# zhenpeiyang/RelativePose

Measured on AMD Instinct MI355X. Metric: scan-pairs/sec end-to-end (completion+feat+spectral-match), 160x640 RGB-D, higher is better.
Workload: dtype f32 (fp32 products emulated on the bf16 matrix pipe: every operand cut into 3 bf16 pieces = its full 24 significand bits, the 6 partial products >= 2^-16 |ab| issued as v_mfma_f32_32x32x16_bf16, the 3 smallest dropped: a product error <= 2^-23 |ab| worst case, rms 2^-27.4 -- an fp32 multiply's own r

## Files before the change

### include/relpose.h

```cpp
#ifndef RELPOSE_H
#define RELPOSE_H

#include <stddef.h>
#include <stdint.h>

#ifdef __cplusplus
extern "C" {
#endif

#define RELPOSE_EINVAL (-1)
#define RELPOSE_ENOMEM (-2)

enum {
    RELPOSE_OK = 0,
    RELPOSE_FEW_KEYPOINTS = 1,
    RELPOSE_DIST_FILTER = 2,
    RELPOSE_ANGLE_FILTER = 3,
    RELPOSE_ZERO_WEIGHT = 4,
    RELPOSE_EDGE_OVERFLOW = 5,
    RELPOSE_NOT_CONVERGED = 6
};

enum { RELPOSE_SUNCG = 0, RELPOSE_MATTERPORT = 1, RELPOSE_SCANNET = 2 };
enum { RELPOSE_MASK_SECOND = 0, RELPOSE_MASK_KINECT = 1 };
enum { RELPOSE_COMPOSE_EVAL = 0, RELPOSE_COMPOSE_LIB = 1 };
enum { RELPOSE_FIT_IRLS_SM = 0, RELPOSE_FIT_HORN87 = 1, RELPOSE_FIT_IRLS = 2, RELPOSE_FIT_SPECTRAL = 3 };

typedef struct RelposeParams {
    double distThre;
    double distSepThre;
    double angleThre;
    double sigmaAngle1, sigmaAngle2, sigmaDist, sigmaFeat;
    double mu;
    int32_t topK;
    int32_t method;
} RelposeParams;

void relpose_default_params(RelposeParams* p_host);

enum { RELPOSE_TUNE_AFFINITY_KERNEL = 0, RELPOSE_TUNE_FIT_MAX_PRODUCTS = 1, RELPOSE_TUNE_FIT_CLUSTER = 2,
       RELPOSE_TUNE_FIT_GLOBAL_VECTORS = 3, RELPOSE_TUNE_FIT_FIXED_CHECKS = 4, RELPOSE_TUNE_HEADS_KERNEL = 5, RELPOSE_TUNE_DECONV_STRIP = 6,
       RELPOSE_TUNE_ZERO_TILES = 7, RELPOSE_TUNE_CONV1_ZERO = 8, RELPOSE_TUNE_COUNT = 9 };
int relpose_set_tuning(int32_t key, int32_t value);
const char* relpose_version(void);
typedef struct RelposeKeypoints {
    int32_t B, ns_max, nt_max;
    const int32_t* ns;
    const int32_t* nt;
    const double* pc_s;
    const double* normal_s;
    const float* feat_s;
    const double* weight_s;
    const double* pc_t;
    const double* normal_t;
    const float* feat_t;
    const double* weight_t;
} RelposeKeypoints;

typedef struct RelposeMatchDebug {
    float* wij;
    int32_t* corres_j;
    double* corres_w;
    int32_t* counts;
    double* trace;
    int32_t* eig_iters;
} RelposeMatchDebug;

#define RELPOSE_MAX_CORRESPONDENCES 8192
#define RELPOSE_MAX_TARGETS 1152
size_t relpose_match_workspace_bytes(int32_t B, int32_t ns_max, int32_t nt_max, int32_t topK, int64_t max_edges);

int relpose_match_pairs(const RelposeParams* params_host, const RelposeKeypoints* kp_host,
                        void* workspace, size_t workspace_bytes, int64_t max_edges,
                        double* pose, int32_t* status, const RelposeMatchDebug* debug_host, void* stream);

typedef struct RelposeMatchArgs {
    uint32_t struct_size;
    int32_t fit_cluster;
    const RelposeParams* params_host;
    const RelposeKeypoints* kp_host;
    void* workspace;
    size_t workspace_bytes;
    int64_t max_edges;
    double* pose;
    int32_t* status;
    const RelposeMatchDebug* debug_host;
    void* stream;
    int32_t affinity_kernel;
    int32_t reserved0;
} RelposeMatchArgs;
int relpose_match_pairs_ex(const RelposeMatchArgs* args);

int relpose_affinity_topk(const RelposeParams* params_host, const RelposeKeypoints* kp_host,
                          float* wij, int32_t* corres_j, double* corres_w, int32_t* k_eff, void* stream);


int relpose_apply_mask(float* x, float* mask, int32_t n, int32_t c, int32_t h, int32_t method, void* stream);

int relpose_build_view(const float* rgb, const float* norm, const float* depth, float* view,
                       int32_t n, int32_t h, int32_t method, void* stream);

int relpose_pano2pc(const float* depth, double* pc, uint8_t* valid, int32_t n, int32_t h, int32_t dataset, void* stream);

size_t relpose_warp_workspace_bytes(int32_t n, int32_t h);
int relpose_warp(const float* view, const double* pose, float* out, void* workspace,
                 int32_t n, int32_t h, int32_t dataset, void* stream);

int relpose_warp_pairs(float* x, const double* pose, void* workspace, int32_t n, int32_t h, int32_t dataset, void* stream);
enum { RELPOSE_WARP_KEYS_CLEAN = 1 };
int relpose_warp_pairs2(float* x, const double* pose, void* workspace, int32_t n, int32_t h, int32_t dataset, int32_t flags, void* stream);

int relpose_pose_inverse(const double* pose, double* inv, int32_t n, void* stream);

int relpose_sample_primitives(const float* f, int32_t cf, int32_t feat_off,
                              const float* obs_norm, const float* obs_depth,
                              const double* pts, const int32_t* npts, int32_t npts_max,
                              double* pc, double* normal, float* feat,
                              int32_t n, int32_t h, int32_t mask_method, int32_t compose, int32_t dataset, void* stream);

int relpose_get_pixel(const double* depth, const double* normal, const double* pts, int32_t k, int32_t h, int32_t dataset,
                      double* pc, double* nn, void* stream);
int relpose_interpolate(const float* feat, const float* pt, float* out, int32_t c, int32_t h, int32_t w, int32_t k, void* stream);

int32_t relpose_observed_points(int32_t h, int32_t dataset);
int relpose_depth2pc(const float* depth, double* pc, uint8_t* valid, int32_t n, int32_t h, int32_t dataset, void* stream);
// ... 388 lines not shown
    int32_t* weight;
    uint32_t* color_sum;
    void* workspace;
    size_t workspace_bytes;
    void* stream;
} RelposeTsdfFuseArgs;
size_t relpose_tsdf_fuse_workspace_bytes(int32_t n_scenes, int32_t n_views, int32_t h, int32_t nx, int32_t ny, int32_t nz);
int relpose_tsdf_fuse(const RelposeTsdfFuseArgs* args);

typedef struct RelposeTsdfSurfaceArgs {
    uint32_t struct_size;
    int32_t n_scenes;
    int32_t nx, ny, nz;
    int32_t min_weight;
    int32_t cap;
    int32_t reserved0;
    const int32_t* tsdf_sum;
    const int32_t* weight;
    const uint32_t* color_sum;
    const double* origin_host;
    double voxel;
    double* points;
    double* normals;
    float* colors;
    uint8_t* valid;
    int32_t* n_points;
    void* workspace;
    size_t workspace_bytes;
    void* stream;
} RelposeTsdfSurfaceArgs;
size_t relpose_tsdf_surface_workspace_bytes(int32_t n_scenes, int32_t nx, int32_t ny, int32_t nz);
int relpose_tsdf_surface(const RelposeTsdfSurfaceArgs* args);

typedef struct RelposeSCNet RelposeSCNet;

RelposeSCNet* relpose_scnet_create(int32_t snumclass, int32_t use_tanh);
void relpose_scnet_destroy(RelposeSCNet* net);

enum { RELPOSE_OUT_RGB = 1, RELPOSE_OUT_N = 2, RELPOSE_OUT_D = 4, RELPOSE_OUT_S = 8, RELPOSE_OUT_F = 16, RELPOSE_OUT_ALL = 31 };
typedef struct RelposeSCNetConfig {
    uint32_t struct_size;
    int32_t snumclass, use_tanh;
    int32_t batchnorm, skip_layer, output_mask;
} RelposeSCNetConfig;
RelposeSCNet* relpose_scnet_create_ex(const RelposeSCNetConfig* cfg);

int relpose_scnet_set_param(RelposeSCNet* net, const char* key, const float* data_host, size_t numel);
int relpose_scnet_finalize(RelposeSCNet* net);
int64_t relpose_scnet_num_params(const RelposeSCNet* net);

enum { RELPOSE_PREC_F32 = 0, RELPOSE_PREC_BF16X3 = 1, RELPOSE_PREC_F16X3 = 2, RELPOSE_PREC_F16 = 3, RELPOSE_PREC_BF16X9 = 4, RELPOSE_PREC_BF16X6 = 5 };
int relpose_scnet_set_precision(RelposeSCNet* net, int32_t mode);

size_t relpose_scnet_workspace_bytes(const RelposeSCNet* net, int32_t n_images, int32_t H, int32_t W);

int relpose_scnet_forward(RelposeSCNet* net, const float* x, float* out, int32_t n_images, int32_t H, int32_t W,
                          void* workspace, size_t workspace_bytes, void* stream);

enum { RELPOSE_FWD_ZERO_WARP = 1, RELPOSE_FWD_POSE_OUTPUTS = 2, RELPOSE_FWD_NEW_WORKSPACE = 4 };
typedef struct RelposeForwardArgs {
    uint32_t struct_size;
    int32_t flags;
    const float* x;
    float* out;
    int32_t n_images, H, W, reserved0;
    void* workspace;
    size_t workspace_bytes;
    void* stream;
    void* tail_stream;
    uint64_t self_tag;
    uint64_t workspace_generation;
    void* reserved1;
} RelposeForwardArgs;
int relpose_scnet_forward_ex(RelposeSCNet* net, const RelposeForwardArgs* args);

int relpose_scnet_plan_macs(RelposeSCNet* net, int32_t n_images, int32_t flags, int32_t self_cached, double* macs_host);

int relpose_scnet_layer_kernel(RelposeSCNet* net, const char* layer, int32_t n_images);

int relpose_scnet_zero_tiles(RelposeSCNet* net, void* workspace, void* stream, int64_t* counts_host);

int relpose_scnet_conv1_zero(RelposeSCNet* net, void* workspace, void* stream, int64_t* counts_host, uint32_t* occ_host);

int64_t relpose_scnet_read_tap(RelposeSCNet* net, const char* layer, float* out, void* workspace, void* stream);

int relpose_scnet_profile(RelposeSCNet* net, const float* x, float* out, int32_t n_images, int32_t H, int32_t W,
                          void* workspace, size_t workspace_bytes, int32_t iters,
                          double* ms_gemm_host, double* ms_other_host, int64_t* n_gemm_launches_host, void* stream);

#ifdef __cplusplus
}
#endif
#endif
```

### relativepose_amd/_lib.py

```python
import ctypes as C
import os

HERE = os.path.dirname(os.path.abspath(__file__))
LIB_PATH = os.environ.get("RELPOSE_LIB_PATH") or os.path.join(HERE, "librelpose_hip.so")

c_void_p, c_int, c_int64, c_size_t, c_double, c_char_p = C.c_void_p, C.c_int32, C.c_int64, C.c_size_t, C.c_double, C.c_char_p


class Params(C.Structure):
    _fields_ = [("distThre", c_double), ("distSepThre", c_double), ("angleThre", c_double),
                ("sigmaAngle1", c_double), ("sigmaAngle2", c_double), ("sigmaDist", c_double),
                ("sigmaFeat", c_double), ("mu", c_double), ("topK", c_int), ("method", c_int)]


class Keypoints(C.Structure):
    _fields_ = [("B", c_int), ("ns_max", c_int), ("nt_max", c_int),
                ("ns", c_void_p), ("nt", c_void_p),
                ("pc_s", c_void_p), ("normal_s", c_void_p), ("feat_s", c_void_p), ("weight_s", c_void_p),
                ("pc_t", c_void_p), ("normal_t", c_void_p), ("feat_t", c_void_p), ("weight_t", c_void_p)]


class MatchDebug(C.Structure):
    _fields_ = [("wij", c_void_p), ("corres_j", c_void_p), ("corres_w", c_void_p),
                ("counts", c_void_p), ("trace", c_void_p), ("eig_iters", c_void_p)]
# ... 160 lines not shown
    _fields_ = [("struct_size", C.c_uint32), ("n_scenes", c_int), ("nx", c_int), ("ny", c_int), ("nz", c_int), ("min_weight", c_int),
                ("cap", c_int), ("reserved0", c_int), ("tsdf_sum", c_void_p), ("weight", c_void_p), ("color_sum", c_void_p),
                ("origin_host", c_void_p), ("voxel", c_double), ("points", c_void_p), ("normals", c_void_p), ("colors", c_void_p),
                ("valid", c_void_p), ("n_points", c_void_p), ("workspace", c_void_p), ("workspace_bytes", c_size_t), ("stream", c_void_p)]


TSDF_MAX_VIEWS = 4096
TSDF_MAX_WEIGHT = 65535


SIGNATURES = {
    "relpose_default_params": (None, [C.POINTER(Params)]),
    "relpose_version": (c_char_p, []),
    "relpose_set_tuning": (c_int, [c_int, c_int]),
    "relpose_match_workspace_bytes": (c_size_t, [c_int, c_int, c_int, c_int, c_int64]),
    "relpose_match_pairs": (c_int, [C.POINTER(Params), C.POINTER(Keypoints), c_void_p, c_size_t, c_int64,
                                    c_void_p, c_void_p, C.POINTER(MatchDebug), c_void_p]),
    "relpose_match_pairs_ex": (c_int, [C.POINTER(MatchArgs)]),
    "relpose_affinity_topk": (c_int, [C.POINTER(Params), C.POINTER(Keypoints), c_void_p, c_void_p, c_void_p, c_void_p, c_void_p]),
    "relpose_apply_mask": (c_int, [c_void_p, c_void_p, c_int, c_int, c_int, c_int, c_void_p]),
    "relpose_build_view": (c_int, [c_void_p, c_void_p, c_void_p, c_void_p, c_int, c_int, c_int, c_void_p]),
    "relpose_pano2pc": (c_int, [c_void_p, c_void_p, c_void_p, c_int, c_int, c_int, c_void_p]),
    "relpose_warp_workspace_bytes": (c_size_t, [c_int, c_int]),
    "relpose_warp": (c_int, [c_void_p, c_void_p, c_void_p, c_void_p, c_int, c_int, c_int, c_void_p]),
    "relpose_warp_pairs": (c_int, [c_void_p, c_void_p, c_void_p, c_int, c_int, c_int, c_void_p]),
    "relpose_warp_pairs2": (c_int, [c_void_p, c_void_p, c_void_p, c_int, c_int, c_int, c_int, c_void_p]),
    "relpose_pose_inverse": (c_int, [c_void_p, c_void_p, c_int, c_void_p]),
    "relpose_sample_primitives": (c_int, [c_void_p, c_int, c_int, c_void_p, c_void_p, c_void_p, c_void_p, c_int,
                                          c_void_p, c_void_p, c_void_p, c_int, c_int, c_int, c_int, c_int, c_void_p]),
    "relpose_get_pixel": (c_int, [c_void_p, c_void_p, c_void_p, c_int, c_int, c_int, c_void_p, c_void_p, c_void_p]),
    "relpose_interpolate": (c_int, [c_void_p, c_void_p, c_void_p, c_int, c_int, c_int, c_int, c_void_p]),
    "relpose_observed_points": (c_int, [c_int, c_int]),
    "relpose_depth2pc": (c_int, [c_void_p, c_void_p, c_void_p, c_int, c_int, c_int, c_void_p]),
    "relpose_depth2pc_full": (c_int, [c_void_p, c_void_p, c_void_p, c_int, c_int, c_int, c_void_p]),
    "relpose_nn_dist": (c_int, [c_void_p, c_void_p, c_int, c_void_p, c_void_p, c_int, c_void_p, c_void_p, c_void_p]),
    "relpose_feature_distance_map": (c_int, [c_void_p, c_void_p, c_void_p, c_int, c_int, c_int, c_void_p]),
    "relpose_nms_sampling": (c_int, [c_void_p, c_void_p, c_int, c_int, c_int, c_int, c_int, c_void_p]),
    "relpose_keypoints_reference_workspace_bytes": (c_size_t, [c_int, c_int, c_int, c_int]),
    "relpose_keypoints_reference": (c_int, [c_void_p, c_int64, c_int, c_int, c_int, c_int, c_void_p, c_void_p, c_void_p, c_void_p, c_int, c_int, c_int, c_int,
                                            c_void_p, c_void_p, c_int, c_int, c_int, c_void_p, c_void_p, c_void_p, c_void_p, c_size_t, c_void_p]),
    "relpose_sift_workspace_bytes": (c_size_t, [c_int, c_int, c_int, c_int]),
    "relpose_sift_stage_capacity": (c_int, [c_int]),
    "relpose_sift_detect": (c_int, [C.POINTER(SiftArgs)]),
    "relpose_fgr_workspace_bytes": (c_size_t, [c_int, c_int, c_int]),
    "relpose_fgr": (c_int, [C.POINTER(FgrArgs)]),
    "relpose_ransac_workspace_bytes": (c_size_t, [c_int, c_int, c_int, c_int, c_int]),
    "relpose_ransac": (c_int, [C.POINTER(RansacArgs)]),
    "relpose_cicp_workspace_bytes": (c_size_t, [c_int, c_int, c_int]),
    "relpose_cicp": (c_int, [C.POINTER(CicpArgs)]),
    "relpose_dense_nn": (c_int, [C.POINTER(DenseNnArgs)]),
    "relpose_descriptor_rank": (c_int, [C.POINTER(DescRankArgs)]),
    "relpose_sift_describe_workspace_bytes": (c_size_t, [c_int, c_int, c_int]),
    "relpose_sift_describe": (c_int, [C.POINTER(SiftDescArgs)]),
    "relpose_sift_rank": (c_int, [C.POINTER(SiftRankArgs)]),
    "relpose_completion_loss_workspace_bytes": (c_size_t, [c_int, c_int, c_int, c_int]),
    "relpose_completion_loss": (c_int, [C.POINTER(CompletionLossArgs)]),
    "relpose_contrast_loss_workspace_bytes": (c_size_t, [c_int, c_int]),
    "relpose_contrast_loss": (c_int, [C.POINTER(ContrastLossArgs)]),
    "relpose_depth_normals": (c_int, [C.POINTER(DepthNormalsArgs)]),
    "relpose_frames_to_pano_workspace_bytes": (c_size_t, [c_int, c_int]),
    "relpose_frames_to_pano": (c_int, [C.POINTER(FramesToPanoArgs)]),
    "relpose_overlap_workspace_bytes": (c_size_t, [c_int, c_int, c_int]),
    "relpose_overlap": (c_int, [C.POINTER(OverlapArgs)]),
    "relpose_visibility_workspace_bytes": (c_size_t, [c_int, c_int, c_int]),
    "relpose_visibility": (c_int, [C.POINTER(VisibilityArgs)]),
    "relpose_tsdf_fuse_workspace_bytes": (c_size_t, [c_int, c_int, c_int, c_int, c_int, c_int]),
    "relpose_tsdf_fuse": (c_int, [C.POINTER(TsdfFuseArgs)]),
    "relpose_tsdf_surface_workspace_bytes": (c_size_t, [c_int, c_int, c_int, c_int]),
    "relpose_tsdf_surface": (c_int, [C.POINTER(TsdfSurfaceArgs)]),
    "relpose_scnet_create": (c_void_p, [c_int, c_int]),
    "relpose_scnet_create_ex": (c_void_p, [C.POINTER(SCNetConfig)]),
    "relpose_scnet_destroy": (None, [c_void_p]),
    "relpose_scnet_set_param": (c_int, [c_void_p, c_char_p, c_void_p, c_size_t]),
    "relpose_scnet_finalize": (c_int, [c_void_p]),
    "relpose_scnet_set_precision": (c_int, [c_void_p, c_int]),
    "relpose_scnet_num_params": (c_int64, [c_void_p]),
    "relpose_scnet_workspace_bytes": (c_size_t, [c_void_p, c_int, c_int, c_int]),
    "relpose_scnet_forward": (c_int, [c_void_p, c_void_p, c_void_p, c_int, c_int, c_int, c_void_p, c_size_t, c_void_p]),
    "relpose_scnet_forward_ex": (c_int, [c_void_p, C.POINTER(ForwardArgs)]),
    "relpose_scnet_plan_macs": (c_int, [c_void_p, c_int, c_int, c_int, C.POINTER(c_double)]),
    "relpose_scnet_layer_kernel": (c_int, [c_void_p, c_char_p, c_int]),
    "relpose_scnet_zero_tiles": (c_int, [c_void_p, c_void_p, c_void_p, C.POINTER(c_int64)]),
    "relpose_scnet_conv1_zero": (c_int, [c_void_p, c_void_p, c_void_p, C.POINTER(c_int64), c_void_p]),
    "relpose_scnet_read_tap": (c_int64, [c_void_p, c_char_p, c_void_p, c_void_p, c_void_p]),
    "relpose_scnet_profile": (c_int, [c_void_p, c_void_p, c_void_p, c_int, c_int, c_int, c_void_p, c_size_t, c_int,
                                      C.POINTER(c_double), C.POINTER(c_double), C.POINTER(c_int64), c_void_p]),
}

_lib = None


def lib():
    global _lib
    if _lib is None:
        if not os.path.exists(LIB_PATH):
            _build_locked()
        if not os.path.exists(LIB_PATH):
            raise RuntimeError(f"{LIB_PATH} not built: run `python -m relativepose_amd.build` "
                               "(or __graft_entry__.build()). There is no CPU fallback.")
        import torch
        l = C.CDLL(LIB_PATH)
        missing = [name for name in SIGNATURES if not hasattr(l, name)]
        if missing:
            raise RuntimeError(f"{LIB_PATH} is stale, missing symbols: {missing}")
        for name, (res, args) in SIGNATURES.items():
            fn = getattr(l, name)
            fn.restype, fn.argtypes = res, args
        _lib = l
    return _lib


def _build_locked():
    import fcntl
    from . import build as _b
    if not os.path.exists(os.environ.get("HIPCC", "/opt/rocm/bin/hipcc")):
        return
    with open(LIB_PATH + ".lock", "w") as lk:
        fcntl.flock(lk, fcntl.LOCK_EX)
        try:
            if not os.path.exists(LIB_PATH):
                _b.build(verbose=False)
        finally:
            fcntl.flock(lk, fcntl.LOCK_UN)


TUNE_KEYS = {"affinity_kernel": 0, "fit_max_products": 1, "fit_cluster": 2, "fit_global_vectors": 3, "fit_fixed_checks": 4,
             "heads_kernel": 5, "deconv_strip": 6, "zero_tiles": 7, "conv1_zero": 8}
AFFINITY_KERNELS = {"auto": 0, "rows": 1, "tile": 2, "lds": 3, "pool": 4}


class tuning:

    def __init__(self, **kw):
        self.kw = {k: (AFFINITY_KERNELS[v] if k == "affinity_kernel" and isinstance(v, str) else int(v)) for k, v in kw.items()}
        self.old = {}

    def __enter__(self):
        for k, v in self.kw.items():
            self.old[k] = lib().relpose_set_tuning(TUNE_KEYS[k], v)
        return self

    def __exit__(self, *exc):
        for k, v in self.old.items():
            lib().relpose_set_tuning(TUNE_KEYS[k], v)
        return False


def check(rc, what):
    if rc != 0:
        raise RuntimeError(f"{what} failed with code {rc}" + (" (HIP error %d)" % (-rc - 1000) if rc <= -1000 else ""))


def require_gpu():
    import torch
    if not torch.cuda.is_available():
        raise RuntimeError("relativepose_amd needs a ROCm GPU (MI355X); there is no CPU fallback")
    return torch.device("cuda", torch.cuda.current_device())


def stream_ptr():
    import torch
    return C.c_void_p(torch.cuda.current_stream().cuda_stream)


def ptr(t):
    return C.c_void_p(t.data_ptr()) if t is not None else C.c_void_p(0)
```

### relativepose_amd/csrc/scnet.hip

```cpp
#include "common.h"
#include "matcher_internal.h"
#include "conv1_zero_geom.h"
#include <map>
#include <string>
#include <vector>
#include <algorithm>
#include <math.h>
#include <stdio.h>
#include <string.h>
#include <type_traits>
#include <stdlib.h>
#include <stddef.h>

namespace {

typedef float floatx16 __attribute__((ext_vector_type(16)));
typedef __bf16 bf16x8 __attribute__((ext_vector_type(8)));
typedef __bf16 bf16x4 __attribute__((ext_vector_type(4)));
typedef _Float16 f16x8 __attribute__((ext_vector_type(8)));
typedef _Float16 f16x4 __attribute__((ext_vector_type(4)));
template <int SPLIT> struct SplitT { typedef bf16x8 v8; typedef bf16x4 v4; };
template <> struct SplitT<2> { typedef f16x8 v8; typedef f16x4 v4; };
template <> struct SplitT<3> { typedef f16x8 v8; typedef f16x4 v4; };
typedef float rp_f4v __attribute__((ext_vector_type(4)));

constexpr int BK = 32;
constexpr int LDK = BK + 4;
constexpr int KQ = BK / 4;
constexpr int LDK3 = 52;
template <int SPLIT> struct RowLd { static constexpr int v = SPLIT >= 4 ? LDK3 : LDK; };
constexpr bool rp_split3(int split) { return split >= 4; }
constexpr float LRELU = 0.1f;
constexpr double BN_EPS = 1e-5;
constexpr int RS = 224;
static_assert(RS == C1Z_RS, "conv1_zero_geom.h");

struct Src {
    const float* x;
    const float2* ss;
    int cstride;
    int C;
    int sstride;
    float slope;
};

struct ConvDesc {
    Src src[2];
    int nsrc, Cin;
    int Nimg, Hin, Win;
    int Hp, Wp, sy, sx;
    int ntaps;
    signed char offy[16], offx[16];
    const float* w;
    int Cout;
    float* y;
    int Hout, Wout, ycstride, ychoff, osy, osx, py, px;
    const float* bias;
    int tanh_out;
    int M, K;
    int ksplit, kt_per;
    int tap_inner;
    float wscale;
    int ntiles_n;
    float* partial;
    double* stat_part;
    int cout_pad;
    int stat_bm;
    int shared_slices;
    int skip_slices;
    int snap_mode;
    float* snap;
    const int* zt_count;
    const int* zt_list;
    const int2* zt_fill;
};

__device__ __forceinline__ float lrelu(float v, float slope) { return fmaxf(v, slope * v); }

typedef float rp_f32x4g __attribute__((__vector_size__(16)));
__device__ __forceinline__ float4 rp_bufld4(__amdgpu_buffer_rsrc_t r, int voff, int soff) {
    const rp_f32x4g f = (rp_f32x4g)__builtin_amdgcn_raw_buffer_load_b128(r, voff, soff, 0);
    return make_float4(f[0], f[1], f[2], f[3]);
}
typedef float rp_f32x2g __attribute__((__vector_size__(8)));
__device__ __forceinline__ float2 rp_bufld2(__amdgpu_buffer_rsrc_t r, int voff, int soff) {
    const rp_f32x2g f = (rp_f32x2g)__builtin_amdgcn_raw_buffer_load_b64(r, voff, soff, 0);
    return make_float2(f[0], f[1]);
}

template <int SPLIT> struct SplitTerms;
template <> struct SplitTerms<1> { static constexpr int NP = 2, NT = 3; static constexpr int ta[3] = {1, 0, 0}, tb[3] = {0, 1, 0}; };
template <> struct SplitTerms<2> { static constexpr int NP = 2, NT = 3; static constexpr int ta[3] = {1, 0, 0}, tb[3] = {0, 1, 0}; };
template <> struct SplitTerms<3> { static constexpr int NP = 1, NT = 1; static constexpr int ta[1] = {0}, tb[1] = {0}; };
template <> struct SplitTerms<4> { static constexpr int NP = 3, NT = 9;
                                   static constexpr int ta[9] = {2, 2, 1, 2, 0, 1, 1, 0, 0}, tb[9] = {2, 1, 2, 0, 2, 1, 0, 1, 0}; };
template <> struct SplitTerms<5> { static constexpr int NP = 3, NT = 6;
                                   static constexpr int ta[6] = {2, 0, 1, 1, 0, 0}, tb[6] = {0, 2, 1, 0, 1, 0}; };
template <int SPLIT>
__device__ __forceinline__ floatx16 rp_mfma16(const typename SplitT<SPLIT>::v8& a, const typename SplitT<SPLIT>::v8& b, const floatx16& c) {
    if constexpr (SPLIT == 2 || SPLIT == 3) return __builtin_amdgcn_mfma_f32_32x32x16_f16(a, b, c, 0, 0, 0);
    else return __builtin_amdgcn_mfma_f32_32x32x16_bf16(a, b, c, 0, 0, 0);
}
template <int SPLIT, int MI, int NI>
__device__ __forceinline__ void rp_split_mma(floatx16 (&acc)[MI][NI], const float* At, const int (&a_rows)[MI], const float* Bt, const int (&b_rows)[NI]) {
    typedef typename SplitT<SPLIT>::v8 h8;
    typedef SplitTerms<SPLIT> TT;
    constexpr int NP = TT::NP, NT = TT::NT;
    {
#pragma unroll
        for (int st = 0; st < 2; ++st) {
            h8 a[NP][MI], b[NP][NI];
#pragma unroll
            for (int pc = 0; pc < NP; ++pc) {
#pragma unroll
                for (int i = 0; i < MI; ++i) a[pc][i] = *reinterpret_cast<const h8*>(&At[a_rows[i] + pc * 16 + st * 8]);
#pragma unroll
                for (int j = 0; j < NI; ++j) b[pc][j] = *reinterpret_cast<const h8*>(&Bt[b_rows[j] + pc * 16 + st * 8]);
            }
#pragma unroll
            for (int t = 0; t < NT; ++t)
#pragma unroll
                for (int i = 0; i < MI; ++i)
#pragma unroll
                    for (int j = 0; j < NI; ++j) acc[i][j] = rp_mfma16<SPLIT>(a[TT::ta[t]][i], b[TT::tb[t]][j], acc[i][j]);
        }
    }
}

template <int WM, int WN, int MI, int NI, bool SSLDS, bool UNI = false, int SPLIT = 0>
__global__ __launch_bounds__(WM * WN * 64, (NI == 4 || SPLIT >= 4) ? 2 : ((WM * WN == 8 || MI == 1) ? 4 : (SSLDS ? 3 : 2))) void conv_igemm_kernel(const ConvDesc* __restrict__ descs, int ninner, int mt_max) {
    constexpr int BM = WM * MI * 32, BN = WN * NI * 32;
    constexpr int LD = RowLd<SPLIT>::v;
    constexpr bool S3 = SPLIT >= 4;
    int zmem, mtile;
    if (ninner == 1) { zmem = blockIdx.x / mt_max; mtile = blockIdx.x - zmem * mt_max; }
    else {
        const int xcd = blockIdx.x & 7, slot = blockIdx.x >> 3, t8 = (mt_max + 7) >> 3;
        const int inner = slot % ninner, rest = slot / ninner;
        zmem = (rest / t8) * ninner + inner;
        mtile = (rest % t8) * 8 + xcd;
    }
    const ConvDesc d = descs[zmem];
    if (mtile * BM >= d.M) return;
    constexpr int NT = WM * WN * 64;
    constexpr int RPI = NT / KQ;
    constexpr int A_IT = BM / RPI;
    constexpr int B_IT = (BN + RPI - 1) / RPI;
    constexpr int SS_CAP = (WN == 2) ? 2048 : 512;
    __shared__ __attribute__((aligned(16))) float As[BM * LD];
    __shared__ __attribute__((aligned(16))) float Bs[BN * LD];
    __shared__ __attribute__((aligned(16))) float sstab[SSLDS ? 2 * SS_CAP : 8];
    __shared__ __attribute__((aligned(16))) int rowpix[BM];
    __shared__ signed char rowslot[BM];
    __shared__ int tapdelta[16];

    const int tid = threadIdx.x, lane = tid & 63, wave = tid >> 6;
    const int wm = wave / WN, wn = wave % WN;
    const int ks = blockIdx.y / d.ntiles_n;
    const int m0 = mtile * BM, n0 = (blockIdx.y - ks * d.ntiles_n) * BN;
    const int hw = d.Hp * d.Wp;
    const int g0 = (m0 / hw) >> 1;

    const int kq = tid % KQ, lrow = tid / KQ;
    int* rtab = reinterpret_cast<int*>(&As[0]);
    for (int row_ = tid; row_ < BM; row_ += NT) {
        const int m = m0 + row_;
        int pix = -1, base = 0, mg = 0, slot = -1;
        if (m < d.M) {
            const int img = m / hw, rem = m - img * hw;
            const int yp = rem / d.Wp, xp = rem - yp * d.Wp;
            pix = (img * d.Hout + yp * d.osy + d.py) * d.Wout + xp * d.osx + d.px;
            slot = min((img >> 1) - g0, 1);
            const int y0 = yp * d.sy, x0 = xp * d.sx;
            base = (img * d.Hin + y0) * d.Win + x0;
            int msk = 0;
            for (int t = 0; t < d.ntaps; ++t) {
                const int iy = y0 + descs[zmem].offy[t], ix = x0 + descs[zmem].offx[t];
                msk |= ((iy >= 0) & (iy < d.Hin) & (ix >= 0) & (ix < d.Win)) ? (1 << t) : 0;
            }
            mg = msk | ((SSLDS ? ((img >> 1) - g0) * d.Cin : (img >> 1)) << 16);
        }
        rowpix[row_] = pix; rowslot[row_] = (signed char)slot;
        rtab[2 * row_] = base; rtab[2 * row_ + 1] = mg;
    }
    if (tid < 16) tapdelta[tid] = (int)descs[zmem].offy[tid] * d.Win + (int)descs[zmem].offx[tid];
    if (SSLDS) {
        const int ng = min(((min(m0 + BM, d.M) - 1) / hw >> 1) - g0 + 1, SS_CAP / d.Cin);
        for (int idx = tid; idx < ng * d.Cin; idx += NT) {
            const int g = g0 + idx / d.Cin, c = idx % d.Cin;
            const bool s1 = c >= d.src[0].C;
            const float2 e = rp_ldg2(reinterpret_cast<const float*>(s1 ? d.src[1].ss + (size_t)g * d.src[1].sstride + (c - d.src[0].C)
                                                                       : d.src[0].ss + (size_t)g * d.src[0].sstride + c));
            sstab[(idx & ~3) * 2 + (idx & 3)] = e.x; sstab[(idx & ~3) * 2 + 4 + (idx & 3)] = e.y;
        }
    }

    floatx16 acc[MI][NI];
#pragma unroll
    for (int i = 0; i < MI; ++i)
#pragma unroll
        for (int j = 0; j < NI; ++j)
#pragma unroll
            for (int r = 0; r < 16; ++r) acc[i][j][r] = 0.f;

    const float* b_src[B_IT];
#pragma unroll
    for (int it = 0; it < B_IT; ++it) {
        const int row = min(lrow + it * RPI, BN - 1);
        b_src[it] = d.w + (size_t)(n0 + row) * d.K * (S3 ? 3 : 2) / 2 + kq * 4;
    }

    int r_base[A_IT], r_mg[UNI ? (A_IT + 1) / 2 : A_IT];
    float4 ra[A_IT], q0[SSLDS ? 1 : A_IT], q1[SSLDS ? 1 : A_IT];
    float4 rb[B_IT];
    float2 rbl[S3 ? B_IT : 1];
#pragma unroll
    for (int it = 0; it < B_IT; ++it) rb[it] = make_float4(0.f, 0.f, 0.f, 0.f);
    static_assert(B_IT <= 8 && (B_IT <= 2 || BN % RPI == 0), "B loader layout");
    int okm = 0, cst = 0;
    const float slope = d.src[0].slope;
    const int kt_begin = ks * d.kt_per;
    const int nkt = min(d.K / BK, kt_begin + d.kt_per);
    const int cpt = d.Cin / BK;
    int tap = d.tap_inner ? kt_begin % d.ntaps : kt_begin / cpt, c0 = (d.tap_inner ? kt_begin / d.ntaps : kt_begin % cpt) * BK;
    __syncthreads();
#pragma unroll
    for (int it = 0; it < A_IT; ++it) {
        const int2 e = *reinterpret_cast<const int2*>(&rtab[2 * (lrow + it * RPI)]);
        r_base[it] = e.x;
        if (!UNI) r_mg[UNI ? 0 : it] = e.y;
        else if (it & 1) r_mg[it >> 1] |= e.y << 16;
        else r_mg[it >> 1] = e.y & 0xffff;
    }

#define RP_ISSUE_LOADS(KT)                                                                                        \
    {                                                                                                             \
        const bool s1_ = (d.nsrc > 1) && (c0 >= d.src[0].C);                                                      \
        const float* sx_ = s1_ ? d.src[1].x : d.src[0].x;                                                         \
        const int scs_ = s1_ ? d.src[1].cstride : d.src[0].cstride;                                               \
        const int cc_ = c0 - (s1_ ? d.src[0].C : 0) + kq * 4;                                                     \
        const int td_ = tapdelta[tap];                                                                            \
        okm = 0; cst = c0 + kq * 4;                                                                               \
        _Pragma("unroll") for (int it = 0; it < A_IT; ++it) {                                                     \
            const bool ok_ = UNI ? ((r_mg[it >> 1] >> (tap + 16 * (it & 1))) & 1) : ((r_mg[UNI ? 0 : it] >> tap) & 1);                                                             \
            okm |= ok_ ? (1 << it) : 0;                                                                           \
            const int pix_ = ok_ ? r_base[it] + td_ : 0;                                                          \
            ra[it] = rp_ldg4(sx_ + (size_t)pix_ * scs_ + cc_);                                                    \
            if (!SSLDS && !UNI) {                                                                                 \
                const float2* sss_ = s1_ ? d.src[1].ss : d.src[0].ss;                                             \
                const int sst_ = s1_ ? d.src[1].sstride : d.src[0].sstride;                                       \
                const float* q = reinterpret_cast<const float*>(sss_ + (size_t)(r_mg[UNI ? 0 : it] >> 16) * sst_ + cc_);      \
                q0[SSLDS ? 0 : it] = rp_ldg4(q); q1[SSLDS ? 0 : it] = rp_ldg4(q + 4);                             \
            }                                                                                                     \
        }                                                                                                         \
        if (!SSLDS && UNI) {                                                                                      \
            const float2* sss_ = s1_ ? d.src[1].ss : d.src[0].ss;                                                 \
            const int sst_ = s1_ ? d.src[1].sstride : d.src[0].sstride;                                           \
            const float* q = reinterpret_cast<const float*>(sss_ + (size_t)g0 * sst_ + cc_);                      \
            qu0 = rp_ldg4(q); qu1 = rp_ldg4(q + 4);                                                               \
        }                                                                                                         \
        const int kof_ = (tap * d.Cin + c0) * (S3 ? 3 : 2) / 2;                                                   \
        _Pragma("unroll") for (int it = 0; it < B_IT; ++it) {                                                     \
            rb[it] = rp_ldg4(b_src[it] + kof_);                                                                   \
            if (S3) { const float2 l_ = rp_ldg2(b_src[it] + kof_ + 32 - kq * 2); rbl[S3 ? it : 0] = l_; }          \
        }                                                                                                         \
        if (d.tap_inner) { ++tap; if (tap == d.ntaps) { tap = 0; c0 += BK; } }                                    \
        else { c0 += BK; if (c0 == d.Cin) { c0 = 0; ++tap; } }                                                    \
    }

#define RP_STORE_TILE()                                                                                           \
    {                                                                                                             \
                                                     \
        float4 u0_ = make_float4(qu0.x, qu0.z, qu1.x, qu1.z), u1_ = make_float4(qu0.y, qu0.w, qu1.y, qu1.w);      \
        if (SSLDS && UNI) {                                                                                       \
            const float4* q = reinterpret_cast<const float4*>(&sstab[2 * cst]);                                   \
            u0_ = q[0]; u1_ = q[1];                                                                               \
        }                                                                                                         \
        const rp_v2f sl2_ = {slope, slope};                                                                       \
        _Pragma("unroll") for (int it = 0; it < A_IT; ++it) {                                                     \
            float4 s0_, s1v_;                                                                                     \
            if (UNI) { s0_ = u0_; s1v_ = u1_; }                                                                   \
            else if (SSLDS) {                                                                                     \
                const float4* q = reinterpret_cast<const float4*>(&sstab[2 * ((r_mg[UNI ? 0 : it] >> 16) + cst)]);          \
                s0_ = q[0]; s1v_ = q[1];                                                                          \
            } else {                                                                                              \
                const float4 a_ = q0[SSLDS ? 0 : it], b_ = q1[SSLDS ? 0 : it];                                    \
                s0_ = make_float4(a_.x, a_.z, b_.x, b_.z); s1v_ = make_float4(a_.y, a_.w, b_.y, b_.w);            \
            }                                                                                                     \
            rp_v2f v01 = {ra[it].x, ra[it].y}, v23 = {ra[it].z, ra[it].w};                                        \
            v01 = v01 * (rp_v2f){s0_.x, s0_.y} + (rp_v2f){s1v_.x, s1v_.y};                                        \
            v23 = v23 * (rp_v2f){s0_.z, s0_.w} + (rp_v2f){s1v_.z, s1v_.w};                                        \
            const rp_v2f t01 = v01 * sl2_, t23 = v23 * sl2_;                                                      \
            const float okf_ = ((okm >> it) & 1) ? 1.f : 0.f;                                                     \
            const rp_v2f mk_ = {okf_, okf_};                                                                      \
            v01 = (rp_v2f){fmaxf(v01.x, t01.x), fmaxf(v01.y, t01.y)} * mk_;                                       \
            v23 = (rp_v2f){fmaxf(v23.x, t23.x), fmaxf(v23.y, t23.y)} * mk_;                                       \
            if (!SPLIT) *reinterpret_cast<float4*>(&As[(lrow + it * RPI) * LD + kq * 4]) = make_float4(v01.x, v01.y, v23.x, v23.y); \
            else {    \
                typedef typename SplitT<SPLIT>::v4 h4_;                                                           \
                const rp_f4v vf_ = {v01.x, v01.y, v23.x, v23.y};                                                  \
                const h4_ hi_ = __builtin_convertvector(vf_, h4_);                                                \
                const rp_f4v r1_ = vf_ - __builtin_convertvector(hi_, rp_f4v);                                    \
                const h4_ lo_ = __builtin_convertvector(r1_, h4_);                                                \
                h4_* ar_ = reinterpret_cast<h4_*>(&As[(lrow + it * RPI) * LD]);                              \
                ar_[kq] = hi_;                                                                                    \
                if (SPLIT != 3) ar_[8 + kq] = lo_;                                                                \
                if (S3) ar_[16 + kq] = __builtin_convertvector(r1_ - __builtin_convertvector(lo_, rp_f4v), h4_);  \
            }                                                                                                     \
        }                                                                                                         \
        if (BN >= RPI || lrow < BN) {                                                                             \
            *reinterpret_cast<float4*>(&Bs[lrow * LD + kq * 4]) = rb[0];                                     \
            if (S3) *reinterpret_cast<float2*>(&Bs[lrow * LD + 32 + kq * 2]) = rbl[0];                       \
        }                                                                                                         \
        _Pragma("unroll") for (int it = 1; it < B_IT; ++it) {                                                     \
            *reinterpret_cast<float4*>(&Bs[(lrow + it * RPI) * LD + kq * 4]) = rb[it];                       \
            if (S3) *reinterpret_cast<float2*>(&Bs[(lrow + it * RPI) * LD + 32 + kq * 2]) = rbl[S3 ? it : 0]; \
        }                                                                                                         \
    }

    float4 qu0 = make_float4(0.f, 0.f, 0.f, 0.f), qu1 = qu0;
    RP_ISSUE_LOADS(kt_begin)
    __syncthreads();
    RP_STORE_TILE()
    __syncthreads();
    const int arow = (wm * MI * 32 + (lane & 31)) * LD + (lane >> 5) * 4;
    const int brow = (wn * NI * 32 + (lane & 31)) * LD + (lane >> 5) * 4;
    for (int kt = kt_begin; kt < nkt; ++kt) {
        if (kt + 1 < nkt) RP_ISSUE_LOADS(kt + 1)
        if constexpr (SPLIT != 0) {
            int ar_[MI], br_[NI];
#pragma unroll
            for (int i = 0; i < MI; ++i) ar_[i] = arow + i * 32 * LD;
#pragma unroll
            for (int j = 0; j < NI; ++j) br_[j] = brow + j * 32 * LD;
            rp_split_mma<SPLIT, MI, NI>(acc, &As[0], ar_, &Bs[0], br_);
        } else
#pragma unroll
        for (int kc = 0; kc < BK / 8; ++kc) {
            float4 a[MI], b[NI];
#pragma unroll
            for (int i = 0; i < MI; ++i) a[i] = *reinterpret_cast<const float4*>(&As[arow + i * 32 * LDK + kc * 8]);
#pragma unroll
            for (int j = 0; j < NI; ++j) b[j] = *reinterpret_cast<const float4*>(&Bs[brow + j * 32 * LDK + kc * 8]);
#pragma unroll
            for (int i = 0; i < MI; ++i)
#pragma unroll
                for (int j = 0; j < NI; ++j) {
                    acc[i][j] = __builtin_amdgcn_mfma_f32_32x32x2f32(a[i].x, b[j].x, acc[i][j], 0, 0, 0);
                    acc[i][j] = __builtin_amdgcn_mfma_f32_32x32x2f32(a[i].y, b[j].y, acc[i][j], 0, 0, 0);
                    acc[i][j] = __builtin_amdgcn_mfma_f32_32x32x2f32(a[i].z, b[j].z, acc[i][j], 0, 0, 0);
                    acc[i][j] = __builtin_amdgcn_mfma_f32_32x32x2f32(a[i].w, b[j].w, acc[i][j], 0, 0, 0);
                }
        }
        __syncthreads();
        if (kt + 1 < nkt) RP_STORE_TILE()
        __syncthreads();
    }
#undef RP_ISSUE_LOADS
#undef RP_STORE_TILE
    if constexpr (SPLIT == 2 || SPLIT == 3) {
#pragma unroll
        for (int i = 0; i < MI; ++i)
#pragma unroll
            for (int j = 0; j < NI; ++j)
#pragma unroll
                for (int r = 0; r < 16; ++r) acc[i][j][r] *= d.wscale;
    }

    if (d.ksplit > 1) {
        float* po = d.partial + (size_t)ks * d.M * d.cout_pad;
#pragma unroll
        for (int i = 0; i < MI; ++i)
#pragma unroll
            for (int r = 0; r < 16; ++r) {
                const int m = m0 + wm * MI * 32 + i * 32 + (r & 3) + 8 * (r >> 2) + 4 * (lane >> 5);
                if (m >= d.M) continue;
#pragma unroll
                for (int j = 0; j < NI; ++j) rp_stg(po + (size_t)m * d.cout_pad + n0 + wn * NI * 32 + j * 32 + (lane & 31), acc[i][j][r]);
            }
        return;
    }
    if (d.stat_part) {
        double* red = reinterpret_cast<double*>(&As[0]);
        double s0[NI], q0s[NI], s1[NI], q1s[NI];
#pragma unroll
        for (int j = 0; j < NI; ++j) { s0[j] = 0; q0s[j] = 0; s1[j] = 0; q1s[j] = 0; }
#pragma unroll
        for (int i = 0; i < MI; ++i)
#pragma unroll
            for (int r = 0; r < 16; ++r) {
                const int sl = UNI ? 0 : rowslot[wm * MI * 32 + i * 32 + (r & 3) + 8 * (r >> 2) + 4 * (lane >> 5)];
#pragma unroll
                for (int j = 0; j < NI; ++j) {
                    const double v = (double)acc[i][j][r];
                    if (UNI) { s0[j] += v; q0s[j] += v * v; }
                    else {
                        const double v0 = sl == 0 ? v : 0.0, v1 = sl == 1 ? v : 0.0;
                        s0[j] += v0; q0s[j] += v0 * v0; s1[j] += v1; q1s[j] += v1 * v1;
                    }
                }
            }
#pragma unroll
        for (int j = 0; j < NI; ++j) {
            s0[j] += rp_shfl_xor_d(s0[j], 32); q0s[j] += rp_shfl_xor_d(q0s[j], 32);
            if (!UNI) { s1[j] += rp_shfl_xor_d(s1[j], 32); q1s[j] += rp_shfl_xor_d(q1s[j], 32); }
            if (lane < 32) {
                const int cl = wn * NI * 32 + j * 32 + lane;
                red[((0 * WM + wm) * BN + cl) * 2 + 0] = s0[j]; red[((0 * WM + wm) * BN + cl) * 2 + 1] = q0s[j];
                red[((1 * WM + wm) * BN + cl) * 2 + 0] = s1[j]; red[((1 * WM + wm) * BN + cl) * 2 + 1] = q1s[j];
            }
        }
        __syncthreads();
        for (int idx = tid; idx < 2 * BN; idx += NT) {
            const int sl = idx / BN, cl = idx - sl * BN;
            double a = 0, b = 0;
#pragma unroll
            for (int w = 0; w < WM; ++w) { a += red[((sl * WM + w) * BN + cl) * 2]; b += red[((sl * WM + w) * BN + cl) * 2 + 1]; }
            double* o = d.stat_part + (((size_t)mtile * 2 + sl) * d.cout_pad + n0 + cl) * 2;
            rp_stg(o, a); rp_stg(o + 1, b);
        }
    }
    const int col0 = n0 + wn * NI * 32 + (lane & 31);
    if (!d.bias && !d.tanh_out) {
#pragma unroll
        for (int i = 0; i < MI; ++i)
#pragma unroll
            for (int r4 = 0; r4 < 4; ++r4) {
                const int4 px = *reinterpret_cast<const int4*>(&rowpix[wm * MI * 32 + i * 32 + 8 * r4 + 4 * (lane >> 5)]);
                const int pxs[4] = {px.x, px.y, px.z, px.w};
#pragma unroll
                for (int rr = 0; rr < 4; ++rr) {
                    if (pxs[rr] < 0) continue;
                    float* yo = d.y + (size_t)pxs[rr] * d.ycstride + d.ychoff + col0;
#pragma unroll
                    for (int j = 0; j < NI; ++j)
                        if (col0 + j * 32 < d.Cout) rp_stg(yo + j * 32, acc[i][j][r4 * 4 + rr]);
                }
            }
        return;
    }
    float bias_v[NI];
#pragma unroll
    for (int j = 0; j < NI; ++j) bias_v[j] = (d.bias && col0 + j * 32 < d.Cout) ? rp_ldg(d.bias + col0 + j * 32) : 0.f;
#pragma unroll
    for (int i = 0; i < MI; ++i)
#pragma unroll
        for (int r = 0; r < 16; ++r) {
            const int pix = rowpix[wm * MI * 32 + i * 32 + (r & 3) + 8 * (r >> 2) + 4 * (lane >> 5)];
            if (pix < 0) continue;
            float* yo = d.y + (size_t)pix * d.ycstride + d.ychoff + col0;
#pragma unroll
            for (int j = 0; j < NI; ++j)
                if (col0 + j * 32 < d.Cout) {
                    float v = acc[i][j][r] + bias_v[j];
                    if (d.tanh_out) v = tanhf(v);
                    rp_stg(yo + j * 32, v);
                }
        }
// ... 910 lines not shown
                        for (int j = 0; j < NI; ++j) {
                            if (pass == 0) { s0[j] = 0; q0s[j] = 0; s1[j] = 0; q1s[j] = 0; }
                            else {
                                const double* c = chain + ((wm * NI + j) * 4) * 64 + lane;
                                s0[j] = c[0]; q0s[j] = c[64]; s1[j] = c[128]; q1s[j] = c[192];
                            }
                        }
#pragma unroll
                        for (int r = 0; r < 16; ++r) {
                            const int m = m0 + 32 * wave + (r & 3) + 8 * (r >> 2) + 4 * h;
                            const int sl = m >= d.M ? -1 : (m >= gb ? 1 : 0);
#pragma unroll
                            for (int j = 0; j < NI; ++j) {
                                const double v = (double)acc[0][j][r];
                                const double v0 = sl == 0 ? v : 0.0, v1 = sl == 1 ? v : 0.0;
                                s0[j] += v0; q0s[j] += v0 * v0; s1[j] += v1; q1s[j] += v1 * v1;
                            }
                        }
#pragma unroll
                        for (int j = 0; j < NI; ++j) {
                            if (pass == 0) {
                                double* c = chain + ((wm * NI + j) * 4) * 64 + lane;
                                c[0] = s0[j]; c[64] = q0s[j]; c[128] = s1[j]; c[192] = q1s[j];
                            } else {
                                s0[j] += rp_shfl_xor_d(s0[j], 32); q0s[j] += rp_shfl_xor_d(q0s[j], 32);
                                s1[j] += rp_shfl_xor_d(s1[j], 32); q1s[j] += rp_shfl_xor_d(q1s[j], 32);
                                if (lane < 32) {
                                    const int cl = j * 32 + lane;
                                    red[((0 * 2 + wm) * 128 + cl) * 2 + 0] = s0[j]; red[((0 * 2 + wm) * 128 + cl) * 2 + 1] = q0s[j];
                                    red[((1 * 2 + wm) * 128 + cl) * 2 + 0] = s1[j]; red[((1 * 2 + wm) * 128 + cl) * 2 + 1] = q1s[j];
                                }
                            }
                        }
                    }
                    __syncthreads();
                }
                {
                    const int sl = tid >> 7, cl = tid & 127;
                    double a = 0, b = 0;
#pragma unroll
                    for (int w = 0; w < 2; ++w) { a += red[((sl * 2 + w) * 128 + cl) * 2]; b += red[((sl * 2 + w) * 128 + cl) * 2 + 1]; }
                    double* o = d.stat_part + (((size_t)mtile * 2 + sl) * d.cout_pad + n0 + cl) * 2;
                    rp_stg(o, a); rp_stg(o + 1, b);
                }
            }
            const int col0 = n0 + l31;
#pragma unroll
            for (int r = 0; r < 16; ++r) {
                const int m = m0 + 32 * wave + (r & 3) + 8 * (r >> 2) + 4 * h;
                if (m >= d.M) continue;
                const int img = m / hw, rem = m - img * hw;
                const int yp = rem / d.Win, xp = rem - yp * d.Win;
                const int pix = (img * d.Hout + yp * d.osy + d.py) * d.Wout + xp * d.osx + d.px;
                float* yo = d.y + (size_t)pix * d.ycstride + d.ychoff + col0;
#pragma unroll
                for (int j = 0; j < NI; ++j)
                    if (col0 + j * 32 < d.Cout) rp_stg(yo + j * 32, acc[0][j][r]);
            }
            return;
        }
    }
    const float wsc = (SPLIT == 2 || SPLIT == 3) ? d.wscale : 1.f;
    float* po = d.partial + (size_t)ks * d.M * d.cout_pad;
#pragma unroll
    for (int r = 0; r < 16; ++r) {
        const int m = m0 + 32 * wave + (r & 3) + 8 * (r >> 2) + 4 * h;
        if (m >= d.M) continue;
#pragma unroll
        for (int j = 0; j < NI; ++j) rp_stg(po + (size_t)m * d.cout_pad + n0 + j * 32 + l31, acc[0][j][r] * wsc);
    }
}

__global__ __launch_bounds__(256) void splitk_reduce_kernel(const ConvDesc* __restrict__ descs) {
    const ConvDesc d = descs[blockIdx.z];
    const int q4 = d.cout_pad >> 2;
    const size_t total = (size_t)d.M * q4;
    const int hw = d.Hp * d.Wp;
    for (size_t idx = (size_t)blockIdx.x * blockDim.x + threadIdx.x; idx < total; idx += (size_t)gridDim.x * blockDim.x) {
        const int m = (int)(idx / q4), c4 = (int)(idx - (size_t)m * q4) * 4;
        float4 a = make_float4(0.f, 0.f, 0.f, 0.f);
        const int img = m / hw, rem = m - img * hw;
        const int msh = (img & 1) * hw + rem;
        for (int ks = 0; ks < d.ksplit; ++ks) {
            const float4 v = rp_ldg4(d.partial + ((size_t)ks * d.M + (((d.shared_slices >> ks) & 1) ? msh : m)) * d.cout_pad + c4);
            a.x += v.x; a.y += v.y; a.z += v.z; a.w += v.w;
        }
        const int yp = rem / d.Wp, xp = rem - yp * d.Wp;
        const size_t pix = ((size_t)img * d.Hout + yp * d.osy + d.py) * d.Wout + xp * d.osx + d.px;
        float* yo = d.y + pix * d.ycstride + d.ychoff + c4;
        if (c4 + 3 < d.Cout) rp_stg4(yo, a);
        else { if (c4 < d.Cout) rp_stg(yo, a.x); if (c4 + 1 < d.Cout) rp_stg(yo + 1, a.y); if (c4 + 2 < d.Cout) rp_stg(yo + 2, a.z); }
    }
}

constexpr int C1_PASSES_PER_GROUP = 2 * RS * RS / 256;
constexpr int C1T_PS = 17;
constexpr int C1T_XIN = 10 * 34 * C1T_PS;
__global__ __launch_bounds__(256, 3) void conv1_mfma_kernel(const float* __restrict__ x0, const float* __restrict__ w1,
                                                          float* __restrict__ a1, double* __restrict__ stat, int n, int mode,
                                                          const unsigned* __restrict__ occ, unsigned char* __restrict__ a1z,
                                                          unsigned short* __restrict__ zcode) {
    __shared__ __attribute__((aligned(16))) float wl[6 * 9 * 4 * 32];
    __shared__ __attribute__((aligned(16))) float xin[C1T_XIN];
    static_assert(C1T_XIN * 4 >= 4 * 192 * 2 * 8, "statistics scratch aliases the input tile");
    static_assert(C1Z_TILES == 196 && C1Z_TPR == 7 && C1Z_TH == 8 && C1Z_TW == 32, "conv1_zero_geom.h describes this kernel's tiles");
    const int tid = threadIdx.x, lane = tid & 63, wave = tid >> 6, h = lane >> 5, l31 = lane & 31;
    const int tile = blockIdx.x % 196, img = blockIdx.x / 196;
    const int ty0 = (tile / 7) * 8, tx0 = (tile % 7) * 32;
    unsigned code = 0u;
    {
        const C1zRange zr = c1z_range(tile);
#pragma unroll
        for (int q = 0; q < 6; ++q) {
            if (((mode & 1) && img >= 2 && (q & 1)) || ((mode & 2) && !(q & 1))) continue;
            unsigned c = 3u;
            if (occ) {
                unsigned any = 0u;
                for (int by = zr.by0; by < zr.by1; ++by) { const unsigned v = occ[c1z_word(img, q, by)]; any |= (v & zr.mask) | (v >> 31); }
                if (!any) c = a1z[c1z_byte(img, q, tile)] ? 1u : 2u;
            }
            code |= c << (2 * q);
        }
    }
    if (!(code & 0xaaau)) {
        if (tid == 0) zcode[blockIdx.x] = (unsigned short)code;
        if (tid < 192) {
            const size_t pass = (size_t)(img >> 1) * C1_PASSES_PER_GROUP + (size_t)(img & 1) * 196 + tile;
            double* o = stat + (pass * 192 + tid) * 2;
            o[0] = 0.0; o[1] = 0.0;
        }
        return;
    }
    for (int i = tid; i < 6 * 9 * 4 * 32 / 4; i += 256) reinterpret_cast<float4*>(wl)[i] = reinterpret_cast<const float4*>(w1)[i];
    for (int i = tid; i < 340 * 4; i += 256) {
        const int p = i >> 2, q4 = i & 3;
        const int py = p / 34, px = p - py * 34;
        const int iy = ty0 + py - 1, ix = tx0 + px - 1;
        float4 v = make_float4(0.f, 0.f, 0.f, 0.f);
        if (iy >= 0 && iy < RS && ix >= 0 && ix < RS) v = *reinterpret_cast<const float4*>(x0 + (((size_t)img * RS + iy) * RS + ix) * 16 + q4 * 4);
        float* d = &xin[p * C1T_PS + q4 * 4];
        d[0] = v.x; d[1] = v.y; d[2] = v.z; d[3] = v.w;
    }
    __syncthreads();
    if (occ && tid == 0) {
        zcode[blockIdx.x] = (unsigned short)code;
#pragma unroll
        for (int q = 0; q < 6; ++q) {
            const unsigned c = (code >> (2 * q)) & 3u;
            if (c >= 2u) a1z[c1z_byte(img, q, tile)] = c == 2u ? 1 : 0;
        }
    }
    typedef float f32x16 __attribute__((ext_vector_type(16)));
    const int pb = ((2 * wave) * 34 + l31) * C1T_PS;
    double st_s[6], st_q[6];
#pragma unroll
    for (int q = 0; q < 6; ++q) {
        const int m = q >> 1, sft = (q & 1) * 8;
        const unsigned zc = (code >> (2 * q)) & 3u;
        if (zc <= 1u) { st_s[q] = 0.0; st_q[q] = 0.0; continue; }
        f32x16 acc0, acc1;
#pragma unroll
        for (int r = 0; r < 16; ++r) { acc0[r] = 0.f; acc1[r] = 0.f; }
        const int nk = (m == 2) ? 9 : 18;
        if (zc == 3u) {
#pragma unroll
        for (int kk = 0; kk < nk; ++kk) {
            const int tap = (m == 2) ? kk : (kk >> 1);
// ... 241 lines not shown
        for (int m = 0; m < 3; ++m) {
            const float4 v = xw[lane * 3 + m];
            a3[2 * m] = (rp_v2f){v.x, v.y}; a3[2 * m + 1] = (rp_v2f){v.z, v.w};
        }
        rp_wave_lds_sync();
    } else {
        if constexpr (POSE) { RP_HS_FETCH_A1(xa, 64) RP_HS_FETCH_A1(xb, 128) } else { RP_HS_FETCH_A1(xa, 0) RP_HS_FETCH_A1(xb, 64) }
        if constexpr (POSE) {
            RP_HS_SKIP(xa, RP_HS_FETCH_D2(xa, 32), 1)
            RP_HS_SKIP(xb, RP_HS_FETCH_D2(xb, 64), 2)
        } else {
            RP_HS_SKIP(xa, RP_HS_FETCH_A1(xa, 128), 0)
            RP_HS_SKIP(xb, RP_HS_FETCH_D2(xb, 0), 1)
            RP_HS_SKIP(xa, RP_HS_FETCH_D2(xa, 32), 2)
        }
        if (hd.snap_mode == 1) {
#pragma unroll
            for (int m = 0; m < 3; ++m) xw[lane * 3 + m] = make_float4(a3[2 * m].x, a3[2 * m].y, a3[2 * m + 1].x, a3[2 * m + 1].y);
            rp_wave_lds_sync();
#pragma unroll
            for (int m = 0; m < 3; ++m) rp_stg4(snw + (m * 64 + lane) * 4, xw[m * 64 + lane]);
            rp_wave_lds_sync();
        }
    }
    if constexpr (POSE) {
        RP_HS_D2(xa, RP_HS_FETCH_D2(xa, 160), 1)
        RP_HS_D2(xb, RP_HS_FETCH_D2(xb, 192), 2)
        RP_HS_LINE(xa, , 160, 2304, 32, 8, af, 0)
        RP_HS_LINE(xb, , 192, 2304 + 32 * 32, 32, 8, af, 0)
    } else {
        RP_HS_D2(xb, RP_HS_FETCH_D2(xb, 64), 0)
        RP_HS_D2(xa, RP_HS_FETCH_D2(xa, 96), 1)
        RP_HS_D2(xb, RP_HS_FETCH_D2(xb, 128), 2)
        RP_HS_LINE(xa, RP_HS_FETCH_D2(xa, 160), 96, 768, 24, 6, as_, 0)
        RP_HS_LINE(xb, RP_HS_FETCH_D2(xb, 192), 128, 768 + 32 * 24, 24, 6, as_, 0)
        RP_HS_LINE(xa, , 160, 2304, 32, 8, af, 0)
        RP_HS_LINE(xb, , 192, 2304 + 32 * 32, 32, 8, af, 0)
    }
#undef RP_HS_SKIP
#undef RP_HS_D2
#undef RP_HS_LINE
#undef RP_HS_FETCH_A1
#undef RP_HS_FETCH_D2
#undef RP_HS_FETCH
    float r[cf + 1];
#pragma unroll
    for (int o = 0; o < 3; ++o) { r[o] = POSE ? 0.f : a3[o >> 1][o & 1] + bl[o]; r[3 + o] = a3[2 + (o >> 1)][o & 1] + bl[3 + o]; }
    r[6] = a3[4].x + bl[6];
#pragma unroll
    for (int o = 0; o < S; ++o) r[7 + o] = POSE ? 0.f : as_[o >> 1][o & 1] + bl[7 + o];
#pragma unroll
    for (int k = 0; k < 32; ++k) { const float v = af[k >> 1][k & 1] + bl[7 + S + k]; r[7 + S + k] = hd.use_tanh ? tanhf(v) : v; }
    float* const xwf = reinterpret_cast<float*>(xw);
#pragma unroll
    for (int h = 0; h < 2; ++h) {
        if ((lane >> 5) == h) {
#pragma unroll
            for (int k = 0; k < cf / 2; ++k) *reinterpret_cast<float2*>(xwf + (lane & 31) * cf + 2 * k) = make_float2(r[2 * k], r[2 * k + 1]);
        }
        rp_wave_lds_sync();
        float* const o = hd.out + (wpix0 + h * 32) * cf;
        for (int i = lane; i < 8 * cf; i += 64) rp_stg4(o + i * 4, xw[i]);
        rp_wave_lds_sync();
    }
}

__global__ __launch_bounds__(256) void splitk_reduce_stats_kernel(const ConvDesc* __restrict__ descs, int nch, int C, double* __restrict__ partial) {
    extern __shared__ __attribute__((aligned(16))) double sm_rs[];
    const ConvDesc d = descs[blockIdx.z];
    const int q4 = d.cout_pad >> 2, nrl = 256 / q4;
    const int cq = threadIdx.x % q4, rl = threadIdx.x / q4;
    const int g = blockIdx.y, chunk = blockIdx.x;
    const int hw = d.Hp * d.Wp, R = 2 * hw;
    const int chunk_rows = (R + nch - 1) / nch;
    const int r0 = g * R + chunk * chunk_rows, r1 = min(min(r0 + chunk_rows, (g + 1) * R), d.M);
    double sv[4] = {0, 0, 0, 0}, qv[4] = {0, 0, 0, 0};
    if (rl < nrl) {
        const int c4 = cq * 4;
        for (int m = r0 + rl; m < r1; m += nrl) {
            float4 a = make_float4(0.f, 0.f, 0.f, 0.f);
            const int img = m / hw, rem = m - img * hw;
            const int msh = (img & 1) * hw + rem;
            for (int ks = 0; ks < d.ksplit; ++ks) {
                const float4 v = rp_ldg4(d.partial + ((size_t)ks * d.M + (((d.shared_slices >> ks) & 1) ? msh : m)) * d.cout_pad + c4);
                a.x += v.x; a.y += v.y; a.z += v.z; a.w += v.w;
            }
            const int yp = rem / d.Wp, xp = rem - yp * d.Wp;
            const size_t pix = ((size_t)img * d.Hout + yp * d.osy + d.py) * d.Wout + xp * d.osx + d.px;
            float* yo = d.y + pix * d.ycstride + d.ychoff + c4;
            if (c4 + 3 < d.Cout) rp_stg4(yo, a);
            else { if (c4 < d.Cout) rp_stg(yo, a.x); if (c4 + 1 < d.Cout) rp_stg(yo + 1, a.y); if (c4 + 2 < d.Cout) rp_stg(yo + 2, a.z); }
            const double e0 = a.x, e1 = a.y, e2 = a.z, e3 = a.w;
            sv[0] += e0; sv[1] += e1; sv[2] += e2; sv[3] += e3;
            qv[0] += e0 * e0; qv[1] += e1 * e1; qv[2] += e2 * e2; qv[3] += e3 * e3;
        }
#pragma unroll
        for (int k = 0; k < 4; ++k) { sm_rs[(rl * q4 + cq) * 8 + k] = sv[k]; sm_rs[(rl * q4 + cq) * 8 + 4 + k] = qv[k]; }
    }
    __syncthreads();
    if (rl == 0) {
        const size_t rec = (size_t)g * (nch * gridDim.z) + blockIdx.z * nch + chunk;
#pragma unroll
        for (int k = 0; k < 4; ++k) {
            const int c = cq * 4 + k;
            if (c >= d.Cout) continue;
            double a = 0, b = 0;
            for (int j = 0; j < nrl; ++j) { a += sm_rs[(j * q4 + cq) * 8 + k]; b += sm_rs[(j * q4 + cq) * 8 + 4 + k]; }
            double* o = partial + (rec * C + d.ychoff + c) * 2;
            o[0] = a; o[1] = b;
        }
    }
}

__global__ __launch_bounds__(256) void bn_partial_kernel(const float* __restrict__ x, int rows_per_group, int C, int chunk_rows,
                                                          double* __restrict__ partial) {
    extern __shared__ __attribute__((aligned(16))) double sm[];
    const int q4 = C >> 2;
    const int nrl = 256 / q4;
    const int cq = threadIdx.x % q4, rl = threadIdx.x / q4;
    const int g = blockIdx.y, chunk = blockIdx.x, nchunks = gridDim.x;
    double s[4] = {0, 0, 0, 0}, ss[4] = {0, 0, 0, 0};
    if (rl < nrl) {
        const int r1 = min((chunk + 1) * chunk_rows, rows_per_group);
        const float* base = x + (size_t)g * rows_per_group * C + cq * 4;
        for (int r = chunk * chunk_rows + rl; r < r1; r += nrl) {
            const float4 v = *reinterpret_cast<const float4*>(base + (size_t)r * C);
            const double a = v.x, b = v.y, c = v.z, d = v.w;
            s[0] += a; s[1] += b; s[2] += c; s[3] += d;
            ss[0] += a * a; ss[1] += b * b; ss[2] += c * c; ss[3] += d * d;
        }
#pragma unroll
        for (int k = 0; k < 4; ++k) { sm[(rl * q4 + cq) * 8 + k] = s[k]; sm[(rl * q4 + cq) * 8 + 4 + k] = ss[k]; }
    }
    __syncthreads();
    if (rl == 0) {
        double* o = partial + (((size_t)g * nchunks + chunk) * C + cq * 4) * 2;
#pragma unroll
        for (int k = 0; k < 4; ++k) {
            double a = 0, b = 0;
            for (int j = 0; j < nrl; ++j) { a += sm[(j * q4 + cq) * 8 + k]; b += sm[(j * q4 + cq) * 8 + 4 + k]; }
            o[k * 2] = a; o[k * 2 + 1] = b;
        }
    }
}

__global__ void bn_finalize_kernel(const double* __restrict__ partial, int nchunks, int C, int rows_per_group,
                                   const float* __restrict__ gamma, const float* __restrict__ beta, float2* __restrict__ ss) {
    const int c = blockIdx.x * blockDim.x + threadIdx.x, g = blockIdx.y;
    if (c >= C) return;
    double s = 0, q = 0;
    for (int k = 0; k < nchunks; ++k) {
        const double* p = partial + (((size_t)g * nchunks + k) * C + c) * 2;
        s += p[0]; q += p[1];
    }
    const double mean = s / rows_per_group;
    double var = q / rows_per_group - mean * mean;
    if (var < 0) var = 0;
    const double sc = (double)gamma[c] / sqrt(var + BN_EPS);
    ss[(size_t)g * C + c] = make_float2((float)sc, (float)((double)beta[c] - mean * sc));
}

__global__ void ss_fill_kernel(int C, int G, const float* __restrict__ gamma, const float* __restrict__ beta, float2* __restrict__ ss) {
    const int i = blockIdx.x * blockDim.x + threadIdx.x;
    if (i >= C * G) return;
    const int c = i % C;
    ss[i] = make_float2(gamma[c], beta[c]);
}
// ... 90 lines not shown
inline size_t c1z_state_bytes(int n) { return (size_t)n * 6 * C1Z_TILES; }
inline size_t zt_ints(int n) { return zt_list_ints(n) + c1z_state_bytes(n) / 4 + (size_t)n * C1Z_TILES / 2; }

__global__ __launch_bounds__(256) void x0_occupancy_kernel(const float* __restrict__ x0, unsigned* __restrict__ occ, int* __restrict__ counts, int c_begin) {
    __shared__ unsigned w[6];
    const int tid = threadIdx.x, img = blockIdx.x / ZT_NB, by = blockIdx.x % ZT_NB;
    if (blockIdx.x == 0 && tid < ZT_HDR) counts[tid] = 0;
    if (tid < 6) w[tid] = 0u;
    __syncthreads();
    unsigned m[6] = {0u, 0u, 0u, 0u, 0u, 0u};
    const uint4* base = reinterpret_cast<const uint4*>(x0 + ((size_t)img * RS + (size_t)by * ZT_BLK) * RS * 16);
    for (int p = tid; p < ZT_BLK * RS; p += 256) {
        const unsigned bit = 1u << ((p % RS) / ZT_BLK);
#pragma unroll
        for (int s = 0; s < 2; ++s) {
            if (8 * s < c_begin) continue;
            const uint4 a = base[(size_t)p * 4 + 2 * s], b = base[(size_t)p * 4 + 2 * s + 1];
            const unsigned k = 0x7fffffffu, c7 = b.w & k;
            const unsigned v[3] = {max(max(a.x & k, a.y & k), max(a.z & k, c7)), max(max(a.w & k, b.x & k), max(b.y & k, c7)), max(b.z & k, c7)};
#pragma unroll
            for (int mm = 0; mm < 3; ++mm)
                if (v[mm]) m[2 * mm + s] |= bit | (v[mm] >= 0x7f800000u ? 0x80000000u : 0u);
        }
    }
#pragma unroll
    for (int q = 0; q < 6; ++q) if (m[q]) atomicOr(&w[q], m[q]);
    __syncthreads();
    if (tid < 6) occ[((size_t)img * 6 + tid) * ZT_NB + by] = w[tid];
}

struct ZtMembers { int nimg[6]; };
__device__ __forceinline__ int zt_edge_class(int p) {
    const int py = p / ZT_NP, px = p - py * ZT_NP;
    return 3 * (py == 0 ? 0 : (py == ZT_NP - 1 ? 2 : 1)) + (px == 0 ? 0 : (px == ZT_NP - 1 ? 2 : 1));
}
__global__ __launch_bounds__(128) void zero_tile_list_kernel(const unsigned* __restrict__ occ, int* __restrict__ zt, ZtMembers mem, int cap) {
    const int g = blockIdx.x, q = blockIdx.y, layer = blockIdx.z, tid = threadIdx.x;
    if (2 * g >= mem.nimg[q]) return;
    __shared__ unsigned ow[2 * ZT_NB];
    __shared__ int red[2 * ZT_PPI], rep[81], comp[2 * ZT_PPI], nonfin, cnt[2], base[2];
    __shared__ int2 fl[2 * ZT_PPI];
    if (tid == 0) nonfin = 0;
    if (tid < 81) rep[tid] = -1;
    __syncthreads();
    if (tid < 2 * ZT_NB) {
        const unsigned v = occ[((size_t)(2 * g + tid / ZT_NB) * 6 + q) * ZT_NB + tid % ZT_NB];
        ow[tid] = v;
        if (v >> 31) nonfin = 1;
    }
    __syncthreads();
    if (tid < 2 * ZT_PPI) {
        const int img = tid / ZT_PPI, p = tid - img * ZT_PPI, py = p / ZT_NP, px = p - py * ZT_NP;
        const int by0 = max(4 * py - 1, 0), by1 = min(4 * py + 5, ZT_NB), bx0 = max(4 * px - 1, 0), bx1 = min(4 * px + 5, ZT_NB);
        const unsigned mask = ((1u << bx1) - 1u) & ~((1u << bx0) - 1u);
        unsigned any = 0u;
        for (int by = by0; by < by1; ++by) any |= ow[img * ZT_NB + by] & mask;
        red[tid] = (any == 0u && !nonfin) ? 1 : 0;
    }
    __syncthreads();
    const int per = layer ? 2 : 1, nu = 2 * ZT_PPI / per;
    if (tid == 0) {
        int nc = 0, nf = 0;
        for (int u = 0; u < nu; ++u) {
            const int p0 = per * u, p1 = p0 + per - 1;
            const int U = g * nu + u;
            int r = -1;
            if (red[p0] && red[p1]) {
                const int key = layer ? zt_edge_class(p0 % ZT_PPI) * 9 + zt_edge_class(p1 % ZT_PPI) : zt_edge_class(p0 % ZT_PPI);
                r = rep[key];
                if (r < 0) rep[key] = U;
            }
            if (r < 0) comp[nc++] = U;
            else fl[nf++] = make_int2(U, r);
        }
        cnt[0] = nc; cnt[1] = nf;
        int* c = zt + (layer * 6 + q) * 2;
        base[0] = atomicAdd(c, nc); base[1] = atomicAdd(c + 1, nf);
    }
    __syncthreads();
    int* list = zt + ZT_HDR + (size_t)(layer * 6 + q) * cap;
    int2* fills = reinterpret_cast<int2*>(zt + ZT_HDR + (size_t)12 * cap) + (size_t)(layer * 6 + q) * cap;
    if (tid < cnt[0] && base[0] + tid < cap) list[base[0] + tid] = comp[tid];
    if (tid < cnt[1] && base[1] + tid < cap) fills[base[1] + tid] = fl[tid];
}

template <bool PAIR>
__global__ __launch_bounds__(256) void zero_tile_fill_kernel(const ConvDesc* __restrict__ descs) {
    const ConvDesc& d = descs[blockIdx.y];
    if (!d.zt_fill || (int)blockIdx.x >= d.zt_count[1]) return;
    const int2 f = d.zt_fill[blockIdx.x];
    constexpr int PR = PAIR ? 8 : 16, PW = PAIR ? 8 : 16, PER = PAIR ? 2 : 1;
    const int tid = threadIdx.x, ppx = d.Wp / PW, ppi = (d.Hp / PR) * ppx, c4n = d.Cout / 4;
    auto at = [&](int unit, int sp, int r, int c) {
        const int qp = PER * unit + sp, img = qp / ppi, prem = qp - img * ppi;
        const size_t pix = ((size_t)img * d.Hout + (prem / ppx) * PR + r) * d.Wout + (prem % ppx) * PW + c;
        return d.y + pix * d.ycstride + d.ychoff;
    };
    for (int i = tid; i < PER * PR * PW * c4n; i += 256) {
        const int c4 = i % c4n, pp = i / c4n, sp = pp / (PR * PW), lp = pp - sp * (PR * PW), r = lp / PW, c = lp - r * PW;
        const float4 v = *reinterpret_cast<const float4*>(at(f.y, sp, r, c) + 4 * c4);
        *reinterpret_cast<float4*>(at(f.x, sp, r, c) + 4 * c4) = v;
    }
    if (d.stat_part && tid < d.cout_pad) {
        const double2 v = *reinterpret_cast<const double2*>(d.stat_part + (((size_t)f.y * 2) * d.cout_pad + tid) * 2);
        *reinterpret_cast<double2*>(d.stat_part + (((size_t)f.x * 2) * d.cout_pad + tid) * 2) = v;
    }
}

__device__ __forceinline__ void lin_coef(int dst, float scale, int in, int& i0, int& i1, float& l0, float& l1) {
    float src = scale * (dst + 0.5f) - 0.5f;
    if (src < 0.f) src = 0.f;
    i0 = (int)src;
    if (i0 > in - 1) i0 = in - 1;
    i1 = i0 + ((i0 < in - 1) ? 1 : 0);
    l1 = src - i0;
    l0 = 1.f - l1;
}

__device__ __forceinline__ void resize_in_pixel(const float* __restrict__ x, float* __restrict__ y, size_t idx, int img, int oy, int ox, int H, int W,
                                                float shh, float sww, int c_begin, float (&out)[16]) {
    int y0, y1, x0, x1; float ly0, ly1, lx0, lx1;
    lin_coef(oy, shh, H, y0, y1, ly0, ly1);
    lin_coef(ox, sww, W, x0, x1, lx0, lx1);
#pragma unroll
    for (int c = 0; c < 16; ++c) {
        if (c < c_begin) continue;
        const float* p = x + ((size_t)img * 16 + c) * H * W;
        out[c] = ly0 * (lx0 * p[(size_t)y0 * W + x0] + lx1 * p[(size_t)y0 * W + x1]) +
                 ly1 * (lx0 * p[(size_t)y1 * W + x0] + lx1 * p[(size_t)y1 * W + x1]);
    }
    float4* o = reinterpret_cast<float4*>(y + idx * 16);
#pragma unroll
    for (int c = 0; c < 4; ++c) if (4 * c >= c_begin) o[c] = make_float4(out[4 * c], out[4 * c + 1], out[4 * c + 2], out[4 * c + 3]);
}

__global__ void resize_in_kernel(const float* __restrict__ x, float* __restrict__ y, int n, int H, int W, int c_begin) {
    const size_t total = (size_t)n * RS * RS;
    const float shh = (float)H / RS, sww = (float)W / RS;
    for (size_t idx = (size_t)blockIdx.x * blockDim.x + threadIdx.x; idx < total; idx += (size_t)gridDim.x * blockDim.x) {
        const int ox = (int)(idx % RS), oy = (int)((idx / RS) % RS), img = (int)(idx / ((size_t)RS * RS));
        float out[16];
        resize_in_pixel(x, y, idx, img, oy, ox, H, W, shh, sww, c_begin, out);
    }
}

__global__ __launch_bounds__(256) void resize_in_occ_kernel(const float* __restrict__ x, float* __restrict__ y, unsigned* __restrict__ occ,
                                                            int* __restrict__ counts, int H, int W, int c_begin) {
    __shared__ unsigned w[6];
    const int tid = threadIdx.x, img = blockIdx.x / ZT_NB, by = blockIdx.x % ZT_NB;
    if (blockIdx.x == 0 && tid < ZT_HDR) counts[tid] = 0;
    if (tid < 6) w[tid] = 0u;
    __syncthreads();
    const float shh = (float)H / RS, sww = (float)W / RS;
    unsigned m[6] = {0u, 0u, 0u, 0u, 0u, 0u};
    for (int p = tid; p < ZT_BLK * RS; p += 256) {
        const int oy = by * ZT_BLK + p / RS, ox = p % RS;
        float out[16];
        resize_in_pixel(x, y, ((size_t)img * RS + oy) * RS + ox, img, oy, ox, H, W, shh, sww, c_begin, out);
        const unsigned bit = 1u << (ox / ZT_BLK);
#pragma unroll
        for (int s = 0; s < 2; ++s) {
            if (8 * s < c_begin) continue;
            const unsigned k = 0x7fffffffu;
            unsigned b[8];
#pragma unroll
            for (int c = 0; c < 8; ++c) b[c] = __float_as_uint(out[8 * s + c]) & k;
// ... 52 lines not shown
        const Seg g = cur;
        if (!g.lds) {
            const int ox = g.ox_first + lane;
            if (ox < W) {
                int x0, x1; float lx0, lx1;
                lin_coef(ox, sww, RS, x0, x1, lx0, lx1);
                const float* r0 = x + ((size_t)g.img * RS + g.y0) * RS * C;
                const float* r1 = x + ((size_t)g.img * RS + g.y1) * RS * C;
                const float* a = r0 + (size_t)x0 * C; const float* b = r0 + (size_t)x1 * C;
                const float* cc = r1 + (size_t)x0 * C; const float* dd = r1 + (size_t)x1 * C;
                float* o = y + (size_t)g.img * C * H * W + (size_t)g.oy * W + ox;
                for (int c = 0; c < C; ++c)
                    o[(size_t)c * H * W] = g.ly0 * (lx0 * a[c] + lx1 * b[c]) + g.ly1 * (lx0 * cc[c] + lx1 * dd[c]);
            }
            if (sidx + step < nseg) { cur = seg_of(sidx + step); if (cur.lds) prefetch(cur); }
            continue;
        }
        const int nf2 = g.width * C / 2;
#pragma unroll
        for (int r = 0; r < 2; ++r) {
            float2* dst = reinterpret_cast<float2*>(srow + r * RO_MAXW * C);
#pragma unroll
            for (int k = 0; k < RO_PF; ++k) { const int i = lane + 64 * k; if (i < nf2) dst[i] = pf[r][k]; }
        }
        if (sidx + step < nseg) { cur = seg_of(sidx + step); if (cur.lds) prefetch(cur); }
        __builtin_amdgcn_fence(__ATOMIC_RELEASE, "workgroup");
        __builtin_amdgcn_wave_barrier();
        __builtin_amdgcn_fence(__ATOMIC_ACQUIRE, "workgroup");
        const int ox = g.ox_first + lane;
        if (ox < W) {
            int x0, x1; float lx0, lx1;
            lin_coef(ox, sww, RS, x0, x1, lx0, lx1);
            const float* a = srow + (x0 - g.sx) * C;
            const float* b = srow + (x1 - g.sx) * C;
            const float* cc = a + RO_MAXW * C;
            const float* dd = b + RO_MAXW * C;
            float* o = y + (size_t)g.img * C * H * W + (size_t)g.oy * W + ox;
            for (int c = 0; c < C; ++c)
                o[(size_t)c * H * W] = g.ly0 * (lx0 * a[c] + lx1 * b[c]) + g.ly1 * (lx0 * cc[c] + lx1 * dd[c]);
        }
        __builtin_amdgcn_wave_barrier();
    }
}

struct Phase {
    int ntaps; signed char offy[16], offx[16];
    int py, px, Hp, Wp;
    size_t w_off;
    size_t ws_off = 0;
    size_t wh_off = 0;
    float wh_scale = 1.f;
    size_t w3_off = 0;
    int K;
};

struct Layer {
    std::string name;
    int kind;
    int cin, cout, k, stride, pad;
    int cout_pad;
    std::vector<Phase> phases;
    size_t bias_off;
};

struct Buf { std::string name; int H, C; size_t off , ss_off, gb_off; };

}

struct RelposeSCNet {
    int S, use_tanh, cf;
    int bn = 1, skip = 1, omask = 31;
    bool variant() const { return !(bn && skip && omask == 31); }
    std::map<std::string, std::vector<float>> params;
    std::map<std::string, std::vector<int64_t>> shapes;
    bool finalized = false;
    int prec = 0;
    int64_t nparams = 0;
    float* d_w = nullptr;
    float* d_gb = nullptr;
    float2* d_ident = nullptr;
    size_t w1_off = 0;
    size_t wh_off = 0, bh_off = 0;
    std::map<std::pair<void*, int>, void*> plans;
    struct SelfState { uint64_t tag = 0, gen = 0; int n = 0, H = 0, W = 0; bool pose_only = false; };
    std::map<void*, SelfState> self_state;
    std::map<std::string, Layer> layers;
    std::map<std::string, Buf> bufs;
    size_t per_image_floats = 0, ss_float2_per_group = 0;
    size_t gb_floats = 0;
    int last_n = 0;
    const int* last_zt_counts = nullptr;
    int64_t last_zt_units[2] = {0, 0};
    bool w1_finite = false;
    struct A1zState { uint64_t gen = 0; int n = 0, H = 0, W = 0; };
    std::map<void*, A1zState> a1z_state;
    int64_t last_c1_units = 0;
    bool last_c1_codes = false, last_occ = false;
    bool profiling = false;
    std::vector<hipEvent_t> ev;
    std::vector<int> ev_kind;
};

namespace {

struct LayerSpec { const char* name; int kind, cin, cout, k, s, p; };

std::vector<LayerSpec> layer_specs(const RelposeSCNet* net) {
    std::vector<LayerSpec> t;
    const int g = 64, S = net->S;
    const int sm = net->skip ? 2 : 1;
    t.push_back({"conv1", 0, 16, 192, 3, 1, 1});
    const char* mods[3] = {"rgb", "n", "d"};
    static std::string names[64];
    int ni = 0;
    for (int m = 0; m < 3; ++m) {
        names[ni] = std::string("conv2") + mods[m]; t.push_back({names[ni++].c_str(), 0, g / 2, g, 4, 2, 1});
        names[ni] = std::string("conv3") + mods[m]; t.push_back({names[ni++].c_str(), 0, g, g * 2, 4, 2, 1});
    }
    t.push_back({"conv4", 0, g * 12, g * 4, 4, 2, 1});
    t.push_back({"conv5", 0, g * 4, g * 8, 4, 2, 1});
    t.push_back({"conv6", 0, g * 8, g * 8, 4, 2, 1});
    t.push_back({"conv7", 0, g * 8, g * 8, 3, 2, 0});
    t.push_back({"conv8", 0, g * 8, g * 8, 3, 1, 1});
    t.push_back({"conv9", 0, g * 8, g * 16, 3, 1, 0});
    t.push_back({"deconv9", 1, g * 16, g * 8, 3, 1, 0});
    t.push_back({"deconv8", 1, g * 8 * sm, g * 8, 3, 1, 1});
    t.push_back({"deconv7", 1, g * 8 * sm, g * 8, 3, 2, 0});
    t.push_back({"deconv6", 1, g * 8 * sm, g * 8, 4, 2, 1});
    t.push_back({"deconv5", 1, g * 8 * sm, g * 4, 4, 2, 1});
    t.push_back({"deconv4", 1, g * 4 * sm, g * 2, 4, 2, 1});
    const int hc[5] = {3, 3, 1, S, 32};
    const char* heads[5] = {"rgb", "n", "d", "s", "f"};
    for (int m = 0; m < 5; ++m) {
        if (!((net->omask >> m) & 1)) continue;
        const bool skip = m < 3;
        names[ni] = std::string("deconv3") + heads[m]; t.push_back({names[ni++].c_str(), 1, skip ? g * 4 : g * 2, g, 4, 2, 1});
        names[ni] = std::string("deconv2") + heads[m]; t.push_back({names[ni++].c_str(), 1, skip ? g * 2 : g, skip ? g / 2 : g, 4, 2, 1});
        names[ni] = std::string("deconv1") + heads[m]; t.push_back({names[ni++].c_str(), 2, g, hc[m], 1, 1, 0});
    }
    return t;
}

int head_of(const std::string& block) {
    if (block.compare(0, 7, "deconv3") && block.compare(0, 7, "deconv2") && block.compare(0, 7, "deconv1")) return -1;
    const std::string h = block.substr(7);
    const char* heads[5] = {"rgb", "n", "d", "s", "f"};
    for (int m = 0; m < 5; ++m) if (h == heads[m]) return m;
    return -1;
}

void conv1_inputs(int m, int s, int* ch, int& n) {
    const int off = s * 8;
    if (m == 0) { ch[0] = off + 0; ch[1] = off + 1; ch[2] = off + 2; ch[3] = off + 7; n = 4; }
    else if (m == 1) { ch[0] = off + 3; ch[1] = off + 4; ch[2] = off + 5; ch[3] = off + 7; n = 4; }
    else { ch[0] = off + 6; ch[1] = off + 7; n = 2; }
}

bool have(RelposeSCNet* net, const std::string& key, size_t numel) {
    auto it = net->params.find(key);
    if (it == net->params.end() || it->second.size() != numel) {
        fprintf(stderr, "relpose_scnet: missing or mis-sized parameter %s (want %zu)\n", key.c_str(), numel);
        return false;
    }
    return true;
}

inline uint16_t f32_to_bf16(float v) {
    uint32_t u; memcpy(&u, &v, 4);
    if ((u & 0x7fffffffu) > 0x7f800000u) return (uint16_t)((u >> 16) | 0x40);
    u += 0x7fffu + ((u >> 16) & 1u);
    return (uint16_t)(u >> 16);
}
inline float bf16_to_f32(uint16_t h) { const uint32_t u = (uint32_t)h << 16; float v; memcpy(&v, &u, 4); return v; }

// ... 96 lines not shown
            ex = std::max(-14, std::min(ex, 24));
            const float up = ldexpf(1.f, ex);
            P.wh_scale = ldexpf(1.f, -ex);
            for (int n_ = 0; n_ < L.cout_pad; ++n_)
                for (int kt = 0; kt < P.K / 32; ++kt)
                    for (int e = 0; e < 32; ++e) {
                        const float v = w[(size_t)n_ * P.K + kt * 32 + e] * up;
                        const _Float16 hi = (_Float16)v;
                        const _Float16 lo = (_Float16)(v - (float)hi);
                        _Float16* o = wh + ((size_t)n_ * P.K + kt * 32) * 2;
                        o[e] = hi; o[32 + e] = lo;
                    }
            P.w3_off = blob.size();
            blob.resize(blob.size() + (size_t)L.cout_pad * P.K * 3 / 2, 0.f);
            w = blob.data() + P.w_off;
            uint16_t* w3 = reinterpret_cast<uint16_t*>(blob.data() + P.w3_off);
            for (int n_ = 0; n_ < L.cout_pad; ++n_)
                for (int kt = 0; kt < P.K / 32; ++kt)
                    for (int e = 0; e < 32; ++e) {
                        const float v = w[(size_t)n_ * P.K + kt * 32 + e];
                        const uint16_t hi = f32_to_bf16(v);
                        const float r1 = v - bf16_to_f32(hi);
                        const uint16_t mid = f32_to_bf16(r1);
                        const uint16_t lo = f32_to_bf16(r1 - bf16_to_f32(mid));
                        uint16_t* o = w3 + ((size_t)n_ * P.K + kt * 32) * 3;
                        o[e] = hi; o[32 + e] = mid; o[64 + e] = lo;
                    }
        }
    net->layers[L.name] = L;
    return 0;
}

struct BufSpec { const char* name; int H, C; };
const BufSpec BUFS[] = {{"X0", 224, 16},  {"A1", 224, 192}, {"A2", 112, 384}, {"A3", 56, 768},  {"A4", 28, 256}, {"A5", 14, 512},
                        {"A6", 7, 512},   {"A7", 3, 512},   {"A8", 3, 512},   {"A9", 1, 1024},  {"D9", 3, 512},  {"D8", 3, 512},
                        {"D7", 7, 512},   {"D6", 14, 512},  {"D5", 28, 256},  {"D4", 56, 128},  {"D3", 112, 320}, {"D2", 224, 224},
                        {"OUT", 224, 0}};

std::vector<std::pair<std::string, int>> bn_blocks(const std::string& b) {
    typedef std::pair<std::string, int> P;
    if (b == "A1") return {P("conv1rgb", 32), P("conv1rgb", 32), P("conv1n", 32), P("conv1n", 32), P("conv1d", 32), P("conv1d", 32)};
    if (b == "A2") return {P("conv2rgb", 64), P("conv2rgb", 64), P("conv2n", 64), P("conv2n", 64), P("conv2d", 64), P("conv2d", 64)};
    if (b == "A3") return {P("conv3rgb", 128), P("conv3rgb", 128), P("conv3n", 128), P("conv3n", 128), P("conv3d", 128), P("conv3d", 128)};
    if (b == "A4") return {P("conv4", 256)};
    if (b == "A5") return {P("conv5", 512)};
    if (b == "A6") return {P("conv6", 512)};
    if (b == "A7") return {P("conv7", 512)};
    if (b == "A8") return {P("conv8", 512)};
    if (b == "A9") return {P("conv9", 1024)};
    if (b == "D9") return {P("deconv9", 512)};
    if (b == "D8") return {P("deconv8", 512)};
    if (b == "D7") return {P("deconv7", 512)};
    if (b == "D6") return {P("deconv6", 512)};
    if (b == "D5") return {P("deconv5", 256)};
    if (b == "D4") return {P("deconv4", 128)};
    if (b == "D3") return {P("deconv3rgb", 64), P("deconv3n", 64), P("deconv3d", 64), P("deconv3s", 64), P("deconv3f", 64)};
    if (b == "D2") return {P("deconv2rgb", 32), P("deconv2n", 32), P("deconv2d", 32), P("deconv2s", 64), P("deconv2f", 64)};
    return {};
}

enum { OP_CONV = 0, OP_REDUCE = 1, OP_STATS = 2, OP_CONV1 = 3, OP_STATS_FUSED = 4, OP_HEADS = 5, OP_DECONV_TILE = 6, OP_CONV_S2 = 7, OP_CONV_STRIP = 8, OP_BCAST = 9, OP_NOP = 10, OP_SS_FILL = 11, OP_ZT_FILL = 12 };
struct Op { int type; int first, count, cfg; dim3 grid; std::string buf; int sslds = 0, uni = 0, split = 0; int ninner = 1, mt_max = 1; int skip_blk = 0; };

struct Plan {
    int n = 0; void* ws = nullptr;
    bool zero_warp = false;
    bool pose_only = false;
    bool self_cached = false;
    size_t persist_floats = 0;
    size_t snap_floats = 0;
    size_t heads_snap_off = 0;
    int snap_mode = 0;
    std::vector<ConvDesc> descs;
    std::vector<Op> ops;
    size_t splitk_floats = 0;
    size_t stat_doubles = 0;
    ConvDesc* d_descs = nullptr;
    int tail_first = -1;
    int head_count = 0;
    hipEvent_t tail_ev = nullptr, head_ev = nullptr;
    bool zt = false;
    int zt_nimg[6] = {0, 0, 0, 0, 0, 0};
    int64_t zt_units[2] = {0, 0};
};

struct Builder {
    RelposeSCNet* net; int n, G;
    float* act; float2* ss; float* splitk; double* statp;
    int pend_first = -1, pend_count = 0, pend_bm = 0; bool pend_ok = true;
    int pend_reduce = -1, pend_groups = 0;
    Plan* plan;
    int rc = 0;
    int group_first = -1;
    bool zero_warp = false;
    bool pose_only = false;
    bool self_cached = false;
    float* persist = nullptr;
    float* snapbuf = nullptr;
    int skip_slices = 0;
    int snap_mode = 0;
    int force_ksplit = 0, shared_slices = 0;
    int nimg = 0;
    std::string probe_layer;
    int probe_desc = -1;
    int* zt = nullptr;
    int zt_layer = -1;

    float* buf(const std::string& b);
    float2* ssb(const std::string& b);
    Src src(const std::string& b, int choff, int C);
    void begin_group() { group_first = (int)plan->descs.size(); }
    void end_group();
    void conv(const std::string& layer, Src s0, const Src* s1, int Hin, const std::string& out, int ochoff);
    void stats(const std::string& b);
};

size_t partial_doubles(int G) { return (size_t)G * std::max(64 * 1024 * 2, C1_PASSES_PER_GROUP * 192 * 2); }
constexpr int MAX_DESCS = 256;

void Builder::stats(const std::string& b) {
    Op o; o.buf = b; o.cfg = 0;
    if (!net->bn) {
        if (pend_first >= 0) for (int i = pend_first; i < pend_first + pend_count; ++i) plan->descs[i].stat_part = nullptr;
        o.type = OP_SS_FILL; o.first = o.count = 0;
        plan->ops.push_back(o);
        pend_first = -1; pend_count = 0; pend_reduce = -1; pend_groups = 0;
        return;
    }
    if (pend_first >= 0 && pend_ok) { o.type = OP_STATS_FUSED; o.first = pend_first; o.count = pend_count; o.cfg = pend_bm; }
    else {
        o.type = OP_STATS; o.first = o.count = 0;
        if (pend_first >= 0) for (int i = pend_first; i < pend_first + pend_count; ++i) plan->descs[i].stat_part = nullptr;
        if (pend_groups == 1 && pend_reduce >= 0) {
            Op& r = plan->ops[pend_reduce];
            const ConvDesc& d = plan->descs[r.first];
            const int R = 2 * d.Hp * d.Wp;
            const int nrl = std::max(1, 256 / (d.cout_pad / 4));
            const int cap = std::max(1, std::min(128, 65536 / (net->bufs[b].C * r.count)));
            int nch = std::min(cap, std::max(1, (R + nrl - 1) / nrl));
            const int chunk_rows = (R + nch - 1) / nch;
            nch = (R + chunk_rows - 1) / chunk_rows;
            if ((size_t)nch * r.count * net->bufs[b].C * 2 <= (size_t)64 * 1024 * 2 && d.cout_pad <= 1024) {
                r.cfg = 1; r.ninner = nch; r.grid = dim3(nch, G, r.count); r.buf = b;
                o.cfg = 3; o.count = nch * r.count;
            }
        }
    }
    plan->ops.push_back(o);
    pend_first = -1; pend_count = 0; pend_reduce = -1; pend_groups = 0;
}

float* Builder::buf(const std::string& b) { return act ? act + net->bufs[b].off * n : nullptr; }
float2* Builder::ssb(const std::string& b) { return ss ? ss + net->bufs[b].ss_off * G : nullptr; }

Src Builder::src(const std::string& b, int choff, int C) {
    const Buf& B = net->bufs[b];
    Src r; r.x = buf(b) + choff; r.cstride = B.C; r.C = C; r.sstride = B.C;
    if (b == "X0") { r.ss = net->d_ident; r.sstride = 0; r.slope = 1.f; }
    else { r.ss = ssb(b) + choff; r.slope = LRELU; }
    return r;
}

void Builder::conv(const std::string& layer, Src s0, const Src* s1, int Hin, const std::string& out, int ochoff) {
    if (rc) return;
    const Layer& L = net->layers[layer];
    const Buf& O = net->bufs[out];
    const int Hout = O.H;
    if (probe_desc < 0 && !probe_layer.empty() && layer == probe_layer) probe_desc = (int)plan->descs.size();
    zt_layer = !layer.compare(0, 5, "conv2") ? 0 : (!layer.compare(0, 5, "conv3") ? 1 : -1);
    for (const Phase& P : L.phases) {
        ConvDesc d;
        memset(&d, 0, sizeof(d));
        d.src[0] = s0; d.nsrc = 1;
        if (s1) { d.src[1] = *s1; d.nsrc = 2; }
        d.Cin = s0.C + (s1 ? s1->C : 0);
        d.Nimg = nimg > 0 ? nimg : n; d.Hin = Hin; d.Win = Hin;
        if (L.kind == 1) {
            d.sy = d.sx = 1; d.osy = d.osx = L.stride; d.py = P.py; d.px = P.px;
            d.Hp = (Hout - P.py + L.stride - 1) / L.stride; d.Wp = (Hout - P.px + L.stride - 1) / L.stride;
        } else {
            d.sy = d.sx = L.stride; d.osy = d.osx = 1; d.py = d.px = 0; d.Hp = Hout; d.Wp = Hout;
        }
        d.ntaps = P.ntaps;
        memcpy(d.offy, P.offy, 16); memcpy(d.offx, P.offx, 16);
        const bool f16w = (net->prec == RELPOSE_PREC_F16X3 || net->prec == RELPOSE_PREC_F16) && P.wh_off;
        d.w = net->d_w + ((net->prec == 1 && P.ws_off) ? P.ws_off : f16w ? P.wh_off : (net->prec >= RELPOSE_PREC_BF16X9 && P.w3_off) ? P.w3_off : P.w_off);
        d.wscale = f16w ? P.wh_scale : 1.f;
        d.Cout = L.cout; d.cout_pad = L.cout_pad;
        d.y = buf(out); d.Hout = Hout; d.Wout = Hout; d.ycstride = (out == "OUT") ? net->cf : O.C; d.ychoff = ochoff;
// ... 86 lines not shown
                 (d.nsrc == 1 || d.src[1].x == d0.src[1].x) && d.Cin == d0.Cin && d.y == d0.y && d.ychoff == d0.ychoff && d.M == plan->descs[first].M &&
                 d.offy[0] == d.offy[1] && d.offy[2] == d.offy[3] && d.offx[0] == d.offx[2] && d.offx[1] == d.offx[3] &&
                 std::abs(d.offy[0] - d.offy[2]) == 1 && std::abs(d.offx[0] - d.offx[1]) == 1 &&
                 std::min(d.offy[0], d.offy[2]) >= -1 && std::max(d.offy[0], d.offy[2]) <= 1 && std::min(d.offx[0], d.offx[1]) >= -1 && std::max(d.offx[0], d.offx[1]) <= 1 &&
                 127 + (127 + d.Win - 1) / d.Win + (d.Win + 1) + (d.Win + 1) + 2 <= 192;
    }
    if (dstrip && min_kt % (4 * ksplit) != 0) dstrip = false;
    size_t pf = 0;
    for (int i = first; i < first + count; ++i) {
        ConvDesc& d = plan->descs[i];
        d.ntiles_n = cp / BNt;
        d.ksplit = ksplit;
        d.kt_per = (d.K / BK + ksplit - 1) / ksplit;
        if (ksplit > 1) {
            float* base = force_ksplit ? persist : splitk;
            d.partial = base ? base + pf : nullptr; pf += (size_t)ksplit * d.M * cp;
        }
    }
    if (force_ksplit) plan->persist_floats = std::max(plan->persist_floats, pf);
    else plan->splitk_floats = std::max(plan->splitk_floats, pf);
    bool fuse = (ksplit == 1);
    for (int i = first; i < first + count; ++i) fuse = fuse && (2 * plan->descs[i].Hp * plan->descs[i].Wp >= BMt) && !plan->descs[i].bias;
    if (pend_first < 0) { pend_first = first; pend_count = 0; pend_bm = BMt; pend_ok = true; }
    pend_count += count;
    ++pend_groups;
    pend_ok = pend_ok && fuse;
    if (fuse) {
        for (int i = first; i < first + count; ++i) {
            ConvDesc& d = plan->descs[i];
            d.stat_bm = BMt;
            const size_t nd = (size_t)((d.M + BMt - 1) / BMt) * 2 * cp * 2;
            d.stat_part = statp ? statp + plan->stat_doubles : (double*)(uintptr_t)8;
            plan->stat_doubles += nd;
        }
    }
    if (s2_cfg >= 0) {
        Op o; o.type = OP_CONV_S2; o.first = first; o.count = count; o.cfg = s2_cfg; o.split = net->prec;
        o.grid = dim3((unsigned)(plan->descs[first].M / BMt), count, 1);
        plan->ops.push_back(o);
        if (zt_layer >= 0) plan->zt_units[zt_layer] += (int64_t)o.grid.x * count;
        if (zt && zt_layer >= 0 && zt_layer == s2_cfg) {
            const int cap = n * ZT_PPI;
            for (int i = first; i < first + count; ++i) {
                ConvDesc& d = plan->descs[i];
                const int q = d.ychoff / d.Cout;
                if (q < 0 || q >= 6 || d.ychoff != q * d.Cout || d.Cout % 4 || (int)o.grid.x > cap || (plan->zt_nimg[q] && plan->zt_nimg[q] != d.Nimg)) { rc = RELPOSE_EINVAL; return; }
                plan->zt_nimg[q] = d.Nimg;
                d.zt_count = zt + (zt_layer * 6 + q) * 2;
                d.zt_list = zt + ZT_HDR + (size_t)(zt_layer * 6 + q) * cap;
                d.zt_fill = reinterpret_cast<const int2*>(zt + ZT_HDR + (size_t)12 * cap) + (size_t)(zt_layer * 6 + q) * cap;
            }
            plan->zt = true;
            Op f = o; f.type = OP_ZT_FILL;
            plan->ops.push_back(f);
        }
        return;
    }
    if (dtile) {
        Op o; o.type = OP_DECONV_TILE; o.first = first; o.count = count; o.cfg = dt_cfg; o.split = net->prec;
        o.grid = dim3((unsigned)(plan->descs[first].M / BMt), count / 4, dt_cfg >= 2 ? cp / 32 : 1);
        if (dt_cfg != 1) {
            for (int i = first; i < first + count; i += 4) {
                ConvDesc& d = plan->descs[i];
                if (d.nsrc != 2) continue;
                const size_t nfl = (size_t)o.grid.x * o.grid.z * 256 * 64;
                d.snap = snapbuf ? snapbuf + plan->snap_floats : nullptr;
                d.snap_mode = snapbuf ? snap_mode : 0;
                plan->snap_floats += nfl;
            }
        }
        plan->ops.push_back(o);
        return;
    }
    {
        const ConvDesc& d = plan->descs[first];
        const int hw = d.Hp * d.Wp;
        bool ok = net->prec != 1 && count == 1 && ksplit > 1 && cfg == 0 && cp % 128 == 0 && d.osy == 1 && d.osx == 1 && d.sy == 2 && d.sx == 2 &&
                  d.ntaps == 16 && d.offy[0] == -1 && d.offx[0] == -1 && d.offy[15] == 2 && d.offx[15] == 2 && d.nsrc == 1 && d.src[0].sstride != 0 && !d.bias &&
                  d.Hin == 2 * d.Hp && d.Win == 2 * d.Wp && hw >= 128;
        ok = ok && 127 + (127 + d.Wp - 1) / d.Wp + (d.Wp + 1) + (d.Wp + 1) + 2 <= 224;
        if (ok) {
            if (shared_slices && (d.Cin / BK) % ksplit == 0) plan->descs[first].shared_slices = shared_slices;
            if (skip_slices && (d.Cin / BK) % ksplit == 0) plan->descs[first].skip_slices = skip_slices;
            Op o; o.type = OP_CONV_STRIP; o.first = first; o.count = 1; o.cfg = 0; o.split = net->prec;
            o.grid = dim3((unsigned)((d.M + 127) / 128), (cp / 128) * ksplit, 1);
            plan->ops.push_back(o);
            Op r; r.type = OP_REDUCE; r.first = first; r.count = count; r.cfg = 0; r.grid = dim3(256, 1, count);
            plan->ops.push_back(r);
            pend_reduce = (int)plan->ops.size() - 1;
            return;
        }
    }
    if (dstrip && ds_sel == 0) {
        const int mt = (plan->descs[first].M + 127) / 128;
        Op o; o.type = OP_CONV_STRIP; o.first = first; o.count = count; o.cfg = 1; o.split = net->prec; o.mt_max = mt;
        o.grid = dim3((unsigned)(((mt + 7) / 8) * 8 * 4), (cp / 128) * ksplit, count / 4);
        plan->ops.push_back(o);
        if (ksplit == 1) return;
        Op r; r.type = OP_REDUCE; r.first = first; r.count = count; r.cfg = 0; r.grid = dim3(256, 1, count);
        plan->ops.push_back(r);
        pend_reduce = (int)plan->ops.size() - 1;
        return;
    }
    Op o; o.type = OP_CONV; o.first = first; o.count = count; o.cfg = cfg;
    o.ninner = 1; o.mt_max = max_mt;
    if (count % 4 == 0) {
        bool ph = true;
        for (int i = first; i < first + count; i += 4)
            for (int k = 1; k < 4; ++k)
                ph = ph && plan->descs[i + k].src[0].x == plan->descs[i].src[0].x && plan->descs[i + k].osy == 2 && plan->descs[i].osy == 2;
        if (ph && max_mt >= 512) o.ninner = 4;
    }
    o.grid = (o.ninner == 1) ? dim3(max_mt * count, (cp / BNt) * ksplit, 1)
                             : dim3(((max_mt + 7) / 8) * 8 * count, (cp / BNt) * ksplit, 1);
    o.sslds = 1; o.uni = 1;
    for (int i = first; i < first + count; ++i) {
        const ConvDesc& d = plan->descs[i];
        const int hw = d.Hp * d.Wp;
        const int ng = (BMt - 1) / (2 * hw) + 2;
        if ((long)ng * d.Cin > ((cfg == 0 || cfg == 7) ? 2048 : 512) || d.src[0].sstride == 0) o.sslds = 0;
        if ((2 * hw) % BMt) o.uni = 0;
    }
    if (!o.sslds) o.uni = 0;
    o.split = net->prec;
    plan->ops.push_back(o);
    if (ksplit > 1) {
        Op r; r.type = OP_REDUCE; r.first = first; r.count = count; r.cfg = 0; r.grid = dim3(256, 1, count);
        plan->ops.push_back(r);
        pend_reduce = (int)plan->ops.size() - 1;
    }
}

void build_plan(RelposeSCNet* net, int n, Builder& R) {
    const char* mods[3] = {"rgb", "n", "d"};
    const char* heads[5] = {"rgb", "n", "d", "s", "f"};
    auto one = [&](const std::string& layer, Src s0, const Src* s1, int Hin, const std::string& out, int ochoff) {
        R.begin_group(); R.conv(layer, s0, s1, Hin, out, ochoff); R.end_group();
    };
    { Op o; o.type = OP_CONV1; o.first = o.count = o.cfg = 0; R.plan->ops.push_back(o); }
    R.stats("A1");
    if (net->bn) R.plan->ops.back().cfg = 1;
    if (R.self_cached) R.plan->ops.back().skip_blk = 32;
    R.plan->head_count = (int)R.plan->ops.size();
    if (R.self_cached) {
        for (int L = 2; L <= 3; ++L) {
            const std::string name = L == 2 ? "conv2" : "conv3", in = L == 2 ? "A1" : "A2", out = L == 2 ? "A2" : "A3";
            const int cin = L == 2 ? 32 : 64, cout = L == 2 ? 64 : 128, Hin = L == 2 ? 224 : 112;
            R.begin_group();
            for (int q = 1; q < 6; q += 2) R.conv(name + mods[q / 2], R.src(in, q * cin, cin), nullptr, Hin, out, q * cout);
            R.end_group();
            R.stats(out);
            if (R.plan->ops.back().type != OP_STATS_FUSED) R.rc = RELPOSE_EINVAL;
            R.plan->ops.back().skip_blk = cout;
        }
    } else if (!R.zero_warp) {
        R.begin_group();
        for (int q = 0; q < 6; ++q) R.conv(std::string("conv2") + mods[q / 2], R.src("A1", q * 32, 32), nullptr, 224, "A2", q * 64);
        R.end_group(); R.stats("A2");
        R.begin_group();
        for (int q = 0; q < 6; ++q) R.conv(std::string("conv3") + mods[q / 2], R.src("A2", q * 64, 64), nullptr, 112, "A3", q * 128);
        R.end_group(); R.stats("A3");
    } else {
        for (int L = 2; L <= 3; ++L) {
            const std::string name = L == 2 ? "conv2" : "conv3", in = L == 2 ? "A1" : "A2", out = L == 2 ? "A2" : "A3";
            const int cin = L == 2 ? 32 : 64, cout = L == 2 ? 64 : 128, Hin = L == 2 ? 224 : 112;
            for (int stream = 0; stream < 2; ++stream) {
// ... 5 lines not shown
            R.nimg = 0;
            R.stats(out);
            if (R.plan->ops.back().type != OP_STATS_FUSED) R.rc = RELPOSE_EINVAL;
        }
        { Op o; o.type = OP_BCAST; o.first = o.count = o.cfg = 0; o.buf = "A3"; R.plan->ops.push_back(o); }
    }
    R.force_ksplit = 6; R.shared_slices = R.zero_warp ? 0x2a : 0;
    R.skip_slices = R.self_cached ? 0x15 : 0;
    const size_t conv4_desc = R.plan->descs.size();
    one("conv4", R.src("A3", 0, 768), nullptr, 56, "A4", 0);
    R.stats("A4");
    R.force_ksplit = 0; R.shared_slices = 0; R.skip_slices = 0;
    if (R.zero_warp && !R.rc && R.plan->descs[conv4_desc].shared_slices)
        for (Op& o : R.plan->ops) if (o.type == OP_BCAST) o.type = OP_NOP;
    one("conv5", R.src("A4", 0, 256), nullptr, 28, "A5", 0); R.stats("A5");
    one("conv6", R.src("A5", 0, 512), nullptr, 14, "A6", 0); R.stats("A6");
    one("conv7", R.src("A6", 0, 512), nullptr, 7, "A7", 0); R.stats("A7");
    one("conv8", R.src("A7", 0, 512), nullptr, 3, "A8", 0); R.stats("A8");
    one("conv9", R.src("A8", 0, 512), nullptr, 3, "A9", 0); R.stats("A9");
    Src sk;
    const Src* skp = net->skip ? &sk : nullptr;
    one("deconv9", R.src("A9", 0, 1024), nullptr, 1, "D9", 0); R.stats("D9");
    sk = R.src("A8", 0, 512); one("deconv8", R.src("D9", 0, 512), skp, 3, "D8", 0); R.stats("D8");
    sk = R.src("A7", 0, 512); one("deconv7", R.src("D8", 0, 512), skp, 3, "D7", 0); R.stats("D7");
    sk = R.src("A6", 0, 512); one("deconv6", R.src("D7", 0, 512), skp, 7, "D6", 0); R.stats("D6");
    sk = R.src("A5", 0, 512); one("deconv5", R.src("D6", 0, 512), skp, 14, "D5", 0); R.stats("D5");
    sk = R.src("A4", 0, 256); one("deconv4", R.src("D5", 0, 256), skp, 28, "D4", 0); R.stats("D4");
    auto wanted = [&](int m) { return ((net->omask >> m) & 1) && (!R.pose_only || (m != 0 && m != 3)); };
    R.begin_group();
    for (int m = 0; m < 5; ++m) {
        if (!wanted(m)) continue;
        if (m < 3) { sk = R.src("A3", 2 * m * 128, 128); R.conv(std::string("deconv3") + heads[m], R.src("D4", 0, 128), &sk, 56, "D3", m * 64); }
        else R.conv(std::string("deconv3") + heads[m], R.src("D4", 0, 128), nullptr, 56, "D3", m * 64);
    }
    R.end_group(); R.stats("D3");
    const int d2off[5] = {0, 32, 64, 96, 160};
    R.begin_group();
    for (int m = 0; m < 3; ++m) if (wanted(m)) { sk = R.src("A2", 2 * m * 64, 64); R.conv(std::string("deconv2") + heads[m], R.src("D3", m * 64, 64), &sk, 112, "D2", d2off[m]); }
    R.end_group();
    R.begin_group();
    for (int m = 3; m < 5; ++m) if (wanted(m)) R.conv(std::string("deconv2") + heads[m], R.src("D3", m * 64, 64), nullptr, 112, "D2", d2off[m]);
    R.end_group(); R.stats("D2");
    R.plan->tail_first = (int)R.plan->ops.size();
    if (net->S != 15 && net->S != 21) {
        if (R.pose_only) R.rc = RELPOSE_EINVAL;
        const int ooff[5] = {0, 3, 6, 7, 7 + net->S};
        for (int cp = 32; cp <= 64; cp *= 2) {
            R.begin_group();
            for (int m = 0; m < 5; ++m) {
                const auto L = net->layers.find(std::string("deconv1") + heads[m]);
                if (!wanted(m) || L == net->layers.end() || L->second.cout_pad != cp) continue;
                if (m < 3) { sk = R.src("A1", 2 * m * 32, 32); R.conv(std::string("deconv1") + heads[m], R.src("D2", d2off[m], 32), &sk, 224, "OUT", ooff[m]); }
                else R.conv(std::string("deconv1") + heads[m], R.src("D2", d2off[m], 64), nullptr, 224, "OUT", ooff[m]);
            }
            R.end_group();
        }
    } else {
        Op o; o.type = OP_HEADS; o.first = o.count = o.cfg = 0; R.plan->ops.push_back(o);
        R.plan->heads_snap_off = R.plan->snap_floats;
        R.plan->snap_floats += (size_t)n * RS * RS * 12;
    }
    (void)n;
}

inline int plan_snap_mode(const Plan& p, int i) {
    for (const Op& op : p.ops)
        if (op.type == OP_DECONV_TILE && i >= op.first && i < op.first + op.count) return p.descs[op.first + ((i - op.first) & ~3)].snap_mode;
    return 0;
}

void free_plan(RelposeSCNet* net) {
    for (auto& kv : net->plans) {
        Plan* p = (Plan*)kv.second;
        if (p->d_descs) (void)hipFree(p->d_descs);
        if (p->tail_ev) (void)hipEventDestroy(p->tail_ev);
        if (p->head_ev) (void)hipEventDestroy(p->head_ev);
        delete p;
    }
    net->plans.clear();
    net->self_state.clear();
    net->a1z_state.clear();
}

struct WsOffsets { size_t act, ss, partial, splitk, statp, persist, snap, zt, total; };

WsOffsets ws_offsets(RelposeSCNet* net, int n) {
    Plan dry;
    Builder B; B.net = net; B.n = n; B.G = n / 2; B.act = nullptr; B.ss = nullptr; B.splitk = nullptr; B.statp = nullptr; B.plan = &dry;
    build_plan(net, n, B);
    WsOffsets o;
    size_t off = 0;
    o.act = off; off += rp_align(net->per_image_floats * n * sizeof(float));
    o.ss = off; off += rp_align(net->ss_float2_per_group * (n / 2) * sizeof(float2));
    o.partial = off; off += rp_align(partial_doubles(n / 2) * sizeof(double));
    o.splitk = off; off += rp_align(dry.splitk_floats * sizeof(float));
    o.statp = off; off += rp_align(dry.stat_doubles * sizeof(double));
    o.persist = off; off += rp_align(dry.persist_floats * sizeof(float));
    o.snap = off; off += rp_align(dry.snap_floats * sizeof(float));
    o.zt = off; off += rp_align(zt_ints(n) * sizeof(int));
    o.total = off;
    return o;
}

}

extern "C" {

RelposeSCNet* relpose_scnet_create(int32_t snumclass, int32_t use_tanh) {
    if (snumclass < 1 || snumclass > 64) return nullptr;
    RelposeSCNet* net = new RelposeSCNet();
    net->S = snumclass; net->use_tanh = use_tanh; net->cf = 7 + snumclass + 32;
    return net;
}

RelposeSCNet* relpose_scnet_create_ex(const RelposeSCNetConfig* cfg) {
    if (!cfg || cfg->struct_size < sizeof(RelposeSCNetConfig)) return nullptr;
    const int om = cfg->output_mask;
    if (om <= 0 || om > 31) return nullptr;
    if (!cfg->skip_layer && (om & (RELPOSE_OUT_RGB | RELPOSE_OUT_N | RELPOSE_OUT_D))) return nullptr;
    RelposeSCNet* net = relpose_scnet_create(cfg->snumclass, cfg->use_tanh);
    if (!net) return nullptr;
    net->bn = cfg->batchnorm ? 1 : 0; net->skip = cfg->skip_layer ? 1 : 0; net->omask = om;
    return net;
}

void relpose_scnet_destroy(RelposeSCNet* net) {
    if (!net) return;
    if (net->d_w) (void)hipFree(net->d_w);
    if (net->d_gb) (void)hipFree(net->d_gb);
    if (net->d_ident) (void)hipFree(net->d_ident);
    free_plan(net);
    delete net;
}

int relpose_scnet_set_param(RelposeSCNet* net, const char* key, const float* data, size_t numel) {
    if (!net || !key || !data) return RELPOSE_EINVAL;
    net->params[key] = std::vector<float>(data, data + numel);
    net->finalized = false;
    free_plan(net);
    return 0;
}

int64_t relpose_scnet_num_params(const RelposeSCNet* net) {
    if (!net) return 0;
    int64_t n = 0;
    for (auto& kv : net->params) n += (int64_t)kv.second.size();
    return n;
}

int relpose_scnet_set_precision(RelposeSCNet* net, int32_t mode) {
    if (!net || mode < RELPOSE_PREC_F32 || mode > RELPOSE_PREC_BF16X6) return RELPOSE_EINVAL;
    if (net->prec != mode) { net->prec = mode; free_plan(net); }
    return 0;
}

int relpose_scnet_finalize(RelposeSCNet* net) {
    if (!net) return RELPOSE_EINVAL;
    free_plan(net);
    std::vector<float> blob;
    net->layers.clear();
    for (const LayerSpec& sp : layer_specs(net)) {
        int rc = pack_layer(net, sp, blob);
        if (rc) return rc;
    }
    {
        net->w1_off = blob.size();
        blob.resize(blob.size() + 6 * 9 * 4 * 32, 0.f);
        float* w1 = blob.data() + net->w1_off;
        const char* mods[3] = {"rgb", "n", "d"};
        for (int m = 0; m < 3; ++m) {
            const int cin_m = m == 2 ? 2 : 4;
            const float* W = net->params[std::string("conv1") + mods[m] + ".0.weight"].data();
            for (int s2 = 0; s2 < 2; ++s2)
                for (int t = 0; t < 9; ++t)
                    for (int c = 0; c < cin_m; ++c)
                        for (int o = 0; o < 32; ++o)
                            w1[(((size_t)(2 * m + s2) * 9 + t) * 4 + c) * 32 + o] = W[((size_t)o * cin_m + c) * 9 + t];
        }
        net->w1_finite = true;
        for (int i = 0; i < 6 * 9 * 4 * 32; ++i) if (!std::isfinite(w1[i])) net->w1_finite = false;
    }
    {
// ... 28 lines not shown
    std::vector<float> gb;
    for (const BufSpec& bs : BUFS) {
        Buf b; b.name = bs.name; b.H = bs.H; b.C = bs.C ? bs.C : net->cf;
        b.off = off; off += (size_t)b.H * b.H * b.C;
        b.ss_off = ssoff; b.gb_off = gboff;
        auto blocks = bn_blocks(b.name);
        if (!blocks.empty()) {
            ssoff += b.C;
            gb.resize(gboff + 2 * (size_t)b.C, 0.f);
            int c = 0;
            for (auto& blk : blocks) {
                const int hm = head_of(blk.first);
                if (hm >= 0 && !((net->omask >> hm) & 1)) { c += blk.second; continue; }
                if (net->bn) {
                    if (!have(net, blk.first + ".1.weight", blk.second) || !have(net, blk.first + ".1.bias", blk.second)) return RELPOSE_EINVAL;
                    memcpy(gb.data() + gboff + c, net->params[blk.first + ".1.weight"].data(), blk.second * sizeof(float));
                    memcpy(gb.data() + gboff + b.C + c, net->params[blk.first + ".1.bias"].data(), blk.second * sizeof(float));
                } else {
                    if (!have(net, blk.first + ".0.bias", blk.second)) return RELPOSE_EINVAL;
                    for (int i = 0; i < blk.second; ++i) gb[gboff + c + i] = 1.f;
                    memcpy(gb.data() + gboff + b.C + c, net->params[blk.first + ".0.bias"].data(), blk.second * sizeof(float));
                }
                c += blk.second;
            }
            if (c != b.C) return RELPOSE_EINVAL;
            gboff += 2 * (size_t)b.C;
        }
        net->bufs[b.name] = b;
    }
    net->per_image_floats = off; net->ss_float2_per_group = ssoff; net->gb_floats = gboff;
    if (net->d_w) { (void)hipFree(net->d_w); net->d_w = nullptr; }
    if (net->d_gb) { (void)hipFree(net->d_gb); net->d_gb = nullptr; }
    RP_HIP(hipMalloc((void**)&net->d_w, blob.size() * sizeof(float)));
    RP_HIP(hipMemcpy(net->d_w, blob.data(), blob.size() * sizeof(float), hipMemcpyHostToDevice));
    RP_HIP(hipMalloc((void**)&net->d_gb, gb.size() * sizeof(float)));
    RP_HIP(hipMemcpy(net->d_gb, gb.data(), gb.size() * sizeof(float), hipMemcpyHostToDevice));
    if (!net->d_ident) {
        float2 id[16];
        for (int i = 0; i < 16; ++i) id[i] = make_float2(1.f, 0.f);
        RP_HIP(hipMalloc((void**)&net->d_ident, sizeof(id)));
        RP_HIP(hipMemcpy(net->d_ident, id, sizeof(id), hipMemcpyHostToDevice));
    }
    net->finalized = true;
    return 0;
}

size_t relpose_scnet_workspace_bytes(const RelposeSCNet* net, int32_t n, int32_t H, int32_t W) {
    if (!net || !net->finalized || n <= 0 || (n & 1) || H <= 0 || W <= 0) return 0;
    return ws_offsets(const_cast<RelposeSCNet*>(net), n).total;
}

static RelposeForwardArgs rp_fwd_args(const float* x, float* out, int32_t n, int32_t H, int32_t W, void* workspace, size_t workspace_bytes, void* stream,
                                      void* tail_stream, int32_t flags, uint64_t self_tag) {
    RelposeForwardArgs a;
    memset(&a, 0, sizeof(a));
    a.struct_size = (uint32_t)sizeof(a); a.flags = flags; a.x = x; a.out = out; a.n_images = n; a.H = H; a.W = W;
    a.workspace = workspace; a.workspace_bytes = workspace_bytes; a.stream = stream; a.tail_stream = tail_stream; a.self_tag = self_tag;
    return a;
}

int relpose_scnet_forward(RelposeSCNet* net, const float* x, float* out, int32_t n, int32_t H, int32_t W, void* workspace,
                          size_t workspace_bytes, void* stream) {
    const RelposeForwardArgs a = rp_fwd_args(x, out, n, H, W, workspace, workspace_bytes, stream, stream, 0, 0);
    return relpose_scnet_forward_ex(net, &a);
}

int relpose_scnet_forward_ex(RelposeSCNet* net, const RelposeForwardArgs* args) {
    if (!net || !args || args->struct_size < offsetof(RelposeForwardArgs, self_tag)) return RELPOSE_EINVAL;
    const float* x = args->x; float* out = args->out;
    const int32_t n = args->n_images, H = args->H, W = args->W, flags = args->flags;
    void* workspace = args->workspace; const size_t workspace_bytes = args->workspace_bytes;
    const bool variant = net->variant();
    void* stream = args->stream; void* tail_stream = (args->tail_stream && !variant) ? args->tail_stream : args->stream;
    const uint64_t self_tag = (!variant && args->struct_size >= offsetof(RelposeForwardArgs, self_tag) + sizeof(uint64_t)) ? args->self_tag : 0;
    const uint64_t ws_gen = args->struct_size >= offsetof(RelposeForwardArgs, workspace_generation) + sizeof(uint64_t) ? args->workspace_generation : 0;
    if (!net->finalized || !x || !out || !workspace || n <= 0 || (n & 1) || H <= 0 || W <= 0 || n >= (1 << 24)) return RELPOSE_EINVAL;
    if (flags & ~(RELPOSE_FWD_ZERO_WARP | RELPOSE_FWD_POSE_OUTPUTS | RELPOSE_FWD_NEW_WORKSPACE)) return RELPOSE_EINVAL;
    if (args->struct_size >= offsetof(RelposeForwardArgs, reserved1) + sizeof(void*) && args->reserved1) return RELPOSE_EINVAL;
    const int G = n / 2;
    const bool zero_warp = (flags & RELPOSE_FWD_ZERO_WARP) && n > 2 && !variant;
    const bool pose_only = (flags & RELPOSE_FWD_POSE_OUTPUTS) != 0 && !variant;
    Plan* plan = nullptr;
    RelposeSCNet::SelfState commit;
    commit.tag = self_tag; commit.n = n; commit.H = H; commit.W = W; commit.pose_only = pose_only; commit.gen = ws_gen;
    if (flags & RELPOSE_FWD_NEW_WORKSPACE) net->self_state.erase(workspace);
    RelposeSCNet::SelfState prev = net->self_state[workspace];
    net->self_state[workspace] = RelposeSCNet::SelfState();
    bool self_cached = self_tag != 0 && prev.tag == self_tag && prev.n == n && prev.H == H && prev.W == W && prev.pose_only == pose_only && !zero_warp &&
                       prev.gen == ws_gen;
    int snap_mode = 0;
    const bool zt_on = g_rp_tune[RELPOSE_TUNE_ZERO_TILES] != 1;
    const int ds_key = ((g_rp_tune[RELPOSE_TUNE_DECONV_STRIP] == 1 ? 1 : 0) << 28) | ((zt_on ? 0 : 1) << 29);
    for (int attempt = 0; attempt < 2 && !plan; ++attempt) {
        snap_mode = self_cached ? 2 : (self_tag != 0 ? 1 : 0);
        const int plan_key = (int)n | (zero_warp ? 1 << 24 : 0) | (pose_only ? 1 << 25 : 0) | (self_cached ? 1 << 26 : 0) | (snap_mode == 1 ? 1 << 27 : 0) | ds_key;
        auto it = net->plans.find(std::make_pair(workspace, plan_key));
        if (it != net->plans.end()) { plan = (Plan*)it->second; break; }
        const WsOffsets o = ws_offsets(net, n);
        if (workspace_bytes < o.total) return RELPOSE_ENOMEM;
        if (net->plans.size() >= 32) {
            free_plan(net);
            self_cached = false;
            snap_mode = self_tag != 0 ? 1 : 0;
        }
        Plan* p = new Plan();
        p->n = n; p->ws = workspace; p->zero_warp = zero_warp; p->pose_only = pose_only; p->self_cached = self_cached;
        char* ws = (char*)workspace;
        Builder B; B.net = net; B.n = n; B.G = G; B.plan = p; B.zero_warp = zero_warp; B.pose_only = pose_only; B.self_cached = self_cached;
        B.act = (float*)(ws + o.act); B.ss = (float2*)(ws + o.ss); B.splitk = (float*)(ws + o.splitk); B.statp = (double*)(ws + o.statp);
        B.persist = (float*)(ws + o.persist);
        B.snapbuf = (float*)(ws + o.snap); B.snap_mode = snap_mode; p->snap_mode = snap_mode;
        B.zt = zt_on ? (int*)(ws + o.zt) + zt_occ_ints(n) : nullptr;
        build_plan(net, n, B);
        if (B.rc) {
            delete p;
            if (self_cached) { self_cached = false; continue; }
            return B.rc;
        }
        RP_HIP(hipMalloc((void**)&p->d_descs, MAX_DESCS * sizeof(ConvDesc)));
        RP_HIP(hipMemcpy(p->d_descs, p->descs.data(), p->descs.size() * sizeof(ConvDesc), hipMemcpyHostToDevice));
        const int key2 = (int)n | (zero_warp ? 1 << 24 : 0) | (pose_only ? 1 << 25 : 0) | (self_cached ? 1 << 26 : 0) | (snap_mode == 1 ? 1 << 27 : 0) | ds_key;
        net->plans[std::make_pair(workspace, key2)] = p;
        plan = p;
    }
    if (!plan) return RELPOSE_EINVAL;
    net->last_n = n;
    const bool two = tail_stream != stream;
    hipStream_t s = (two && plan->head_count > 0) ? (hipStream_t)tail_stream : (hipStream_t)stream;
    const WsOffsets o = ws_offsets(net, n);
    char* ws = (char*)workspace;
    float* act = (float*)(ws + o.act);
    float2* ssp = (float2*)(ws + o.ss);
    double* partial = (double*)(ws + o.partial);
    auto mark = [&](int kind) {
        if (!net->profiling) return;
        hipEvent_t e; (void)hipEventCreate(&e); (void)hipEventRecord(e, s);
        net->ev.push_back(e); net->ev_kind.push_back(kind);
    };
    if (net->omask != 31) {
        for (const char* bn_ : {"D3", "D2", "OUT"}) {
            const Buf& B = net->bufs[bn_];
            RP_HIP(hipMemsetAsync(act + B.off * n, 0, (size_t)n * B.H * B.H * B.C * sizeof(float), s));
        }
    }
    unsigned* const occ = (unsigned*)(ws + o.zt);
    int* const ztp = (int*)(ws + o.zt) + zt_occ_ints(n);
    unsigned char* const a1z = (unsigned char*)((int*)(ws + o.zt) + zt_list_ints(n));
    unsigned short* const zcode = (unsigned short*)(a1z + c1z_state_bytes(n));
    const bool occ_fused = plan->zt && g_rp_tune[RELPOSE_TUNE_CONV1_ZERO] != 1;
    const bool c1z = occ_fused && net->w1_finite;
    RelposeSCNet::A1zState a1z_prev;
    {
        auto it = net->a1z_state.find(workspace);
        if (it != net->a1z_state.end()) { a1z_prev = it->second; net->a1z_state.erase(it); }
    }
    if (c1z && !(ws_gen != 0 && !(flags & RELPOSE_FWD_NEW_WORKSPACE) && a1z_prev.gen == ws_gen && a1z_prev.n == n && a1z_prev.H == H && a1z_prev.W == W))
        RP_HIP(hipMemsetAsync(a1z, 0, c1z_state_bytes(n), s));
    mark(3);
    if (occ_fused)
        hipLaunchKernelGGL(resize_in_occ_kernel, dim3(n * ZT_NB), dim3(256), 0, s, x, act + net->bufs["X0"].off * n, occ, ztp, H, W, plan->self_cached ? 8 : 0);
    else
        hipLaunchKernelGGL(resize_in_kernel, dim3(2048), dim3(256), 0, s, x, act + net->bufs["X0"].off * n, n, H, W, plan->self_cached ? 8 : 0);
    mark(-3);
    net->last_zt_counts = nullptr;
    net->last_zt_units[0] = plan->zt_units[0]; net->last_zt_units[1] = plan->zt_units[1];
    net->last_c1_units = 0; net->last_c1_codes = false; net->last_occ = plan->zt;
    if (plan->zt) {
        ZtMembers zm;
        for (int q = 0; q < 6; ++q) zm.nimg[q] = plan->zt_nimg[q];
        mark(2);
        if (!occ_fused)
            hipLaunchKernelGGL(x0_occupancy_kernel, dim3(n * ZT_NB), dim3(256), 0, s, act + net->bufs["X0"].off * n, occ, ztp, plan->self_cached ? 8 : 0);
        hipLaunchKernelGGL(zero_tile_list_kernel, dim3(G, 6, 2), dim3(128), 0, s, occ, ztp, zm, n * ZT_PPI);
        mark(-2);
        net->last_zt_counts = ztp;
    }
    int op_index = -1;
    for (const Op& op : plan->ops) {
        ++op_index;
        if (op.type == OP_NOP) continue;
        if (op_index == plan->head_count && s != (hipStream_t)stream) {
            if (!plan->head_ev) RP_HIP(hipEventCreateWithFlags(&plan->head_ev, hipEventDisableTiming));
            RP_HIP(hipEventRecord(plan->head_ev, s));
            s = (hipStream_t)stream;
            RP_HIP(hipStreamWaitEvent(s, plan->head_ev, 0));
        }
        if (op_index == plan->tail_first && two) {
            if (!plan->tail_ev) RP_HIP(hipEventCreateWithFlags(&plan->tail_ev, hipEventDisableTiming));
            RP_HIP(hipEventRecord(plan->tail_ev, s));
            s = (hipStream_t)tail_stream;
            RP_HIP(hipStreamWaitEvent(s, plan->tail_ev, 0));
        }
        if (op.type == OP_CONV) {
            mark(1);
            const ConvDesc* dd = plan->d_descs + op.first;
#define RP_LAUNCH_V(WM_, WN_, MI_, NI_, SS_, UNI_, SP_) \
            hipLaunchKernelGGL((conv_igemm_kernel<WM_, WN_, MI_, NI_, SS_, UNI_, SP_>), op.grid, dim3(256), 0, s, dd, op.ninner, op.mt_max)
#define RP_LAUNCH_T(WM_, WN_, MI_, NI_)                                                                        \
            do {                                                                                               \
                if (op.split == 1) {                                                                           \
                    if (op.uni) RP_LAUNCH_V(WM_, WN_, MI_, NI_, true, true, 1);                                \
                    else if (op.sslds) RP_LAUNCH_V(WM_, WN_, MI_, NI_, true, false, 1);                        \
                    else RP_LAUNCH_V(WM_, WN_, MI_, NI_, false, false, 1);                                     \
                } else if (op.split == 2) {                                                                    \
                    if (op.uni) RP_LAUNCH_V(WM_, WN_, MI_, NI_, true, true, 2);                                \
                    else if (op.sslds) RP_LAUNCH_V(WM_, WN_, MI_, NI_, true, false, 2);                        \
                    else RP_LAUNCH_V(WM_, WN_, MI_, NI_, false, false, 2);                                     \
                } else if (op.split == 3) {                                                                    \
                    if (op.uni) RP_LAUNCH_V(WM_, WN_, MI_, NI_, true, true, 3);                                \
                    else if (op.sslds) RP_LAUNCH_V(WM_, WN_, MI_, NI_, true, false, 3);                        \
                    else RP_LAUNCH_V(WM_, WN_, MI_, NI_, false, false, 3);                                     \
                } else if (op.split == 4) {                                                                    \
                    if (op.uni) RP_LAUNCH_V(WM_, WN_, MI_, NI_, true, true, 4);                                \
                    else if (op.sslds) RP_LAUNCH_V(WM_, WN_, MI_, NI_, true, false, 4);                        \
                    else RP_LAUNCH_V(WM_, WN_, MI_, NI_, false, false, 4);                                     \
                } else if (op.split == 5) {                                                                    \
                    if (op.uni) RP_LAUNCH_V(WM_, WN_, MI_, NI_, true, true, 5);                                \
                    else if (op.sslds) RP_LAUNCH_V(WM_, WN_, MI_, NI_, true, false, 5);                        \
                    else RP_LAUNCH_V(WM_, WN_, MI_, NI_, false, false, 5);                                     \
                } else {                                                                                       \
                    if (op.uni) RP_LAUNCH_V(WM_, WN_, MI_, NI_, true, true, 0);                                \
                    else if (op.sslds) RP_LAUNCH_V(WM_, WN_, MI_, NI_, true, false, 0);                        \
                    else RP_LAUNCH_V(WM_, WN_, MI_, NI_, false, false, 0);                                     \
                }                                                                                              \
            } while (0)
            if (op.cfg == 0) RP_LAUNCH_T(2, 2, 2, 2);
            else if (op.cfg == 1) RP_LAUNCH_T(4, 1, 2, 2);
            else if (op.cfg == 2) RP_LAUNCH_T(4, 1, 2, 1);
            else if (op.cfg == 4) RP_LAUNCH_T(4, 1, 1, 2);
            else if (op.cfg == 7) RP_LAUNCH_T(2, 2, 1, 1);
            else RP_LAUNCH_T(4, 1, 1, 1);
#undef RP_LAUNCH_T
#undef RP_LAUNCH_V
            mark(-1);
        } else if (op.type == OP_CONV_STRIP) {
            mark(1);
#define RP_TILE_SPLIT(LAUNCH_)                                            \
            do {                                                          \
                if (op.split == 2) { LAUNCH_(2); }                        \
                else if (op.split == 3) { LAUNCH_(3); }                   \
                else if (op.split == 4) { LAUNCH_(4); }                   \
                else if (op.split == 5) { LAUNCH_(5); }                   \
                else { LAUNCH_(0); }                                      \
            } while (0)
#define RP_L_STRIP(SP_) hipLaunchKernelGGL((conv_s2_strip_kernel<4, SP_>), op.grid, dim3(256), 0, s, plan->d_descs + op.first)
#define RP_L_DSTRIP(SP_) hipLaunchKernelGGL((deconv_strip_kernel<4, SP_>), op.grid, dim3(256), 0, s, plan->d_descs + op.first, op.mt_max)
            if (op.cfg == 1) RP_TILE_SPLIT(RP_L_DSTRIP);
            else RP_TILE_SPLIT(RP_L_STRIP);
#undef RP_L_STRIP
#undef RP_L_DSTRIP
            mark(-1);
        } else if (op.type == OP_CONV_S2) {
            mark(1);
#define RP_L_S2A(SP_) hipLaunchKernelGGL((conv_s2_tile_kernel<2, 2, 16, false, SP_>), op.grid, dim3(256), 0, s, plan->d_descs + op.first)
#define RP_L_S2C(SP_) hipLaunchKernelGGL((conv_s2_tile_kernel<1, 4, 8, true, SP_>), op.grid, dim3(256), 0, s, plan->d_descs + op.first)
            if (op.cfg == 0) RP_TILE_SPLIT(RP_L_S2A);
            else RP_TILE_SPLIT(RP_L_S2C);
#undef RP_L_S2A
#undef RP_L_S2C
            mark(-1);
        } else if (op.type == OP_ZT_FILL) {
            mark(2);
            if (op.cfg == 0) hipLaunchKernelGGL((zero_tile_fill_kernel<false>), op.grid, dim3(256), 0, s, plan->d_descs + op.first);
            else hipLaunchKernelGGL((zero_tile_fill_kernel<true>), op.grid, dim3(256), 0, s, plan->d_descs + op.first);
            mark(-2);
        } else if (op.type == OP_DECONV_TILE) {
            mark(1);
#define RP_L_DT1(SP_) hipLaunchKernelGGL((deconv_tile_kernel<1, 2, 4, 16, false, SP_>), op.grid, dim3(256), 0, s, plan->d_descs + op.first)
#define RP_L_DT2(SP_) hipLaunchKernelGGL((deconv_tile_kernel<1, 1, 4, 16, false, SP_>), op.grid, dim3(256), 0, s, plan->d_descs + op.first)
#define RP_L_DT4(SP_) hipLaunchKernelGGL((deconv_tile_kernel<1, 1, 4, 8, true, SP_>), op.grid, dim3(256), 0, s, plan->d_descs + op.first)
            if (op.cfg == 1) {
                if (op.split == 2) RP_L_DT1(2);
                else if (op.split == 3) RP_L_DT1(3);
                else if (op.split >= 4) return RELPOSE_EINVAL;
                else RP_L_DT1(0);
            }
            else if (op.cfg == 2) RP_TILE_SPLIT(RP_L_DT2);
            else RP_TILE_SPLIT(RP_L_DT4);
#undef RP_L_DT1
#undef RP_L_DT2
#undef RP_L_DT4
#undef RP_TILE_SPLIT
            mark(-1);
        } else if (op.type == OP_CONV1) {
            mark(1);
            hipLaunchKernelGGL(conv1_mfma_kernel, dim3(196 * n), dim3(256), 0, s, act + net->bufs["X0"].off * n, net->d_w + net->w1_off,
                               act + net->bufs["A1"].off * n, partial, n, (plan->zero_warp ? 1 : 0) | (plan->self_cached ? 2 : 0),
                               c1z ? (const unsigned*)occ : nullptr, a1z, zcode);
            net->last_c1_units = (int64_t)C1Z_TILES * (plan->self_cached ? 3 * n : (plan->zero_warp ? 3 * n + 3 * 2 : 6 * n));
            net->last_c1_codes = c1z;
            mark(-1);
        } else if (op.type == OP_STATS_FUSED) {
            const Buf& B = net->bufs[op.buf];
            mark(2);
            hipLaunchKernelGGL(bn_finalize_fused_kernel, dim3((B.C + 31) / 32, G), dim3(1024), 0, s, plan->d_descs + op.first, op.count, op.skip_blk,
                               B.C, 2 * B.H * B.H, net->d_gb + B.gb_off, net->d_gb + B.gb_off + B.C, ssp + B.ss_off * G);
            mark(-2);
        } else if (op.type == OP_SS_FILL) {
            const Buf& B = net->bufs[op.buf];
            mark(2);
            hipLaunchKernelGGL(ss_fill_kernel, dim3((B.C * G + 255) / 256), dim3(256), 0, s, B.C, G, net->d_gb + B.gb_off, net->d_gb + B.gb_off + B.C,
                               ssp + B.ss_off * G);
            mark(-2);
        } else if (op.type == OP_BCAST) {
            const Buf& B = net->bufs[op.buf];
            mark(2);
            hipLaunchKernelGGL(bcast_warped_kernel, dim3(2048), dim3(256), 0, s, act + B.off * n, n, B.H * B.H, B.C, B.C / 6, ssp + B.ss_off * G, G);
            mark(-2);
        } else if (op.type == OP_HEADS) {
            HeadsDesc hd;
            hd.d2 = act + net->bufs["D2"].off * n; hd.a1 = act + net->bufs["A1"].off * n;
            hd.ss_d2 = ssp + net->bufs["D2"].ss_off * G; hd.ss_a1 = ssp + net->bufs["A1"].ss_off * G;
            hd.w = net->d_w + net->wh_off; hd.bias = net->d_w + net->bh_off; hd.out = act + net->bufs["OUT"].off * n;
            hd.n = n; hd.S = net->S; hd.cf = net->cf; hd.use_tanh = net->use_tanh;
            hd.snap_mode = plan->snap_mode; hd.snap = (float*)(ws + o.snap) + plan->heads_snap_off;
            mark(1);
            const dim3 hg((unsigned)((size_t)n * RS * RS / 256));
#define RP_HEADS_LAUNCH(S_, POSE_)                                                                                         \
            { if (lanepix) hipLaunchKernelGGL((heads_lanepix_kernel<S_, POSE_>), hg, dim3(256), 0, s, hd);               \
              else hipLaunchKernelGGL((heads_kernel<S_, POSE_>), hg, dim3(256), 0, s, hd); }
            const bool lanepix = g_rp_tune[RELPOSE_TUNE_HEADS_KERNEL] == 1;
            if (plan->pose_only) {
                if (net->S == 15) RP_HEADS_LAUNCH(15, true) else RP_HEADS_LAUNCH(21, true)
            } else if (net->S == 15) RP_HEADS_LAUNCH(15, false) else RP_HEADS_LAUNCH(21, false)
#undef RP_HEADS_LAUNCH
            mark(-1);
        } else if (op.type == OP_REDUCE) {
            mark(4);
            if (op.cfg == 1) {
                const ConvDesc& d0 = plan->descs[op.first];
                const int q4 = d0.cout_pad / 4, nrl = 256 / q4;
// ... 48 lines not shown
    return 0;
}

int relpose_scnet_plan_macs(RelposeSCNet* net, int32_t n, int32_t flags, int32_t self_cached, double* macs_out) {
    if (!net || !net->finalized || !macs_out || n <= 0 || (n & 1)) return RELPOSE_EINVAL;
    if (net->variant()) { flags = 0; self_cached = 0; }
    const bool zero_warp = (flags & RELPOSE_FWD_ZERO_WARP) && n > 2 && !self_cached;
    const bool pose_only = (flags & RELPOSE_FWD_POSE_OUTPUTS) != 0;
    Plan dry;
    Builder B; B.net = net; B.n = n; B.G = n / 2; B.act = nullptr; B.ss = nullptr; B.splitk = nullptr; B.statp = nullptr; B.plan = &dry;
    B.zero_warp = zero_warp; B.pose_only = pose_only; B.self_cached = self_cached != 0;
    B.snapbuf = (float*)(uintptr_t)4096;
    B.snap_mode = self_cached ? 2 : 1; dry.snap_mode = B.snap_mode;
    build_plan(net, n, B);
    if (B.rc) return B.rc;
    double macs = 0;
    for (const Op& op : dry.ops) {
        if (op.type == OP_CONV || op.type == OP_CONV_S2 || op.type == OP_CONV_STRIP || op.type == OP_DECONV_TILE) {
            for (int i = op.first; i < op.first + op.count; ++i) {
                const ConvDesc& d = dry.descs[i];
                double rowsK;
                if (op.type == OP_CONV_STRIP && d.ksplit > 1 && (d.shared_slices || d.skip_slices)) {
                    rowsK = 0;
                    for (int ks = 0; ks < d.ksplit; ++ks) {
                        if ((d.skip_slices >> ks) & 1) continue;
                        const double rows = ((d.shared_slices >> ks) & 1) ? 2.0 * d.Hp * d.Wp : (double)d.M;
                        rowsK += rows * d.K / d.ksplit;
                    }
                } else if (op.type == OP_DECONV_TILE && d.nsrc == 2 && plan_snap_mode(dry, i) == 2) {
                    rowsK = (double)d.M * d.ntaps * d.src[0].C;
                } else rowsK = (double)d.M * d.K;
                macs += rowsK * d.Cout;
            }
        } else if (op.type == OP_CONV1) {
            const double blk = 224.0 * 224 * 32 * (36 + 36 + 18);
            const double self_imgs = self_cached ? 0 : n, warp_imgs = zero_warp ? 2 : n;
            macs += blk * (self_imgs + warp_imgs);
        } else if (op.type == OP_HEADS) {
            const double px = (double)n * 224 * 224;
            const int hc[5] = {3, 3, 1, net->S, 32};
            for (int m = 0; m < 5; ++m) {
                if (pose_only && (m == 0 || m == 3)) continue;
                const int cin = (m < 3 && self_cached) ? 32 : 64;
                macs += px * cin * hc[m];
            }
        }
    }
    *macs_out = macs;
    return 0;
}

int relpose_scnet_layer_kernel(RelposeSCNet* net, const char* layer, int32_t n) {
    if (!net || !net->finalized || !layer || n <= 0 || (n & 1)) return RELPOSE_EINVAL;
    Plan dry;
    Builder B; B.net = net; B.n = n; B.G = n / 2; B.act = nullptr; B.ss = nullptr; B.splitk = nullptr; B.statp = nullptr; B.plan = &dry;
    B.probe_layer = layer;
    build_plan(net, n, B);
    if (B.rc) return B.rc;
    if (B.probe_desc < 0) return RELPOSE_EINVAL;
    for (const Op& op : dry.ops)
        if ((op.type == OP_CONV || op.type == OP_CONV_S2 || op.type == OP_CONV_STRIP || op.type == OP_DECONV_TILE) && B.probe_desc >= op.first &&
            B.probe_desc < op.first + op.count)
            return (op.type == OP_CONV_STRIP && op.cfg == 1) ? (dry.descs[B.probe_desc].ksplit == 1 ? 2 : 1) : 0;
    return RELPOSE_EINVAL;
}

int relpose_scnet_zero_tiles(RelposeSCNet* net, void* workspace, void* stream, int64_t* counts_host) {
    if (!net || !net->finalized || !workspace || !counts_host || net->last_n <= 0) return RELPOSE_EINVAL;
    for (int l = 0; l < 2; ++l) { counts_host[2 * l] = net->last_zt_units[l]; counts_host[2 * l + 1] = 0; }
    if (!net->last_zt_counts) return 0;
    const char* lo = (const char*)workspace + ws_offsets(net, net->last_n).zt;
    if ((const char*)net->last_zt_counts < lo || (const char*)net->last_zt_counts >= lo + zt_ints(net->last_n) * sizeof(int)) return RELPOSE_EINVAL;
    int h[ZT_HDR];
    RP_HIP(hipMemcpyAsync(h, net->last_zt_counts, sizeof(h), hipMemcpyDeviceToHost, (hipStream_t)stream));
    RP_HIP(hipStreamSynchronize((hipStream_t)stream));
    for (int l = 0; l < 2; ++l) {
        int64_t c = 0, f = 0;
        for (int q = 0; q < 6; ++q) { c += h[(l * 6 + q) * 2]; f += h[(l * 6 + q) * 2 + 1]; }
        counts_host[2 * l] = c; counts_host[2 * l + 1] = f;
    }
    return 0;
}

int relpose_scnet_conv1_zero(RelposeSCNet* net, void* workspace, void* stream, int64_t* counts_host, uint32_t* occ_host) {
    if (!net || !net->finalized || !workspace || !counts_host || net->last_n <= 0) return RELPOSE_EINVAL;
    const int n = net->last_n;
    counts_host[0] = net->last_c1_units; counts_host[1] = 0; counts_host[2] = 0;
    if (occ_host && !net->last_occ) return RELPOSE_EINVAL;
    const int* base = (const int*)((const char*)workspace + ws_offsets(net, n).zt);
    std::vector<unsigned short> codes;
    if (net->last_c1_codes) {
        codes.resize((size_t)n * C1Z_TILES);
        const unsigned char* a1z = (const unsigned char*)(base + zt_list_ints(n));
        RP_HIP(hipMemcpyAsync(codes.data(), a1z + c1z_state_bytes(n), codes.size() * sizeof(unsigned short), hipMemcpyDeviceToHost, (hipStream_t)stream));
    }
    if (occ_host) RP_HIP(hipMemcpyAsync(occ_host, base, zt_occ_ints(n) * sizeof(uint32_t), hipMemcpyDeviceToHost, (hipStream_t)stream));
    RP_HIP(hipStreamSynchronize((hipStream_t)stream));
    int64_t launched = 0;
    for (unsigned short c : codes)
        for (int q = 0; q < 6; ++q) {
            const int v = (c >> (2 * q)) & 3;
            launched += v != 0; counts_host[1] += v == 1; counts_host[2] += v == 2;
        }
    if (net->last_c1_codes && launched != net->last_c1_units) return RELPOSE_EINVAL;
    return 0;
}

int64_t relpose_scnet_read_tap(RelposeSCNet* net, const char* name, float* out, void* workspace, void* stream) {
    if (!net || !net->finalized || !name || net->last_n <= 0) return -1;
    auto it = net->bufs.find(name);
    if (it == net->bufs.end()) return -1;
    const Buf& B = it->second;
    const int64_t count = (int64_t)net->last_n * B.H * B.H * B.C;
    if (out) {
        if (!workspace) return -1;
        const float* src = (const float*)workspace + B.off * net->last_n;
        if (hipMemcpyAsync(out, src, count * sizeof(float), hipMemcpyDeviceToDevice, (hipStream_t)stream) != hipSuccess) return -1;
    }
    return count;
}

int relpose_scnet_profile(RelposeSCNet* net, const float* x, float* out, int32_t n, int32_t H, int32_t W, void* workspace,
                          size_t workspace_bytes, int32_t iters, double* ms_gemm, double* ms_other, int64_t* n_gemm, void* stream) {
    if (!net || iters <= 0) return RELPOSE_EINVAL;
    double tg = 0, to = 0; int64_t ng = 0;
    for (int it = 0; it < iters; ++it) {
        net->profiling = true; net->ev.clear(); net->ev_kind.clear();
        int rc = relpose_scnet_forward(net, x, out, n, H, W, workspace, workspace_bytes, stream);
        net->profiling = false;
        if (rc) return rc;
        RP_HIP(hipStreamSynchronize((hipStream_t)stream));
        for (size_t i = 0; i + 1 < net->ev.size(); i += 2) {
            float ms = 0;
            if (hipEventElapsedTime(&ms, net->ev[i], net->ev[i + 1]) != hipSuccess) ms = 0.f;
            if (net->ev_kind[i] == 1) { tg += ms; ++ng; } else to += ms;
        }
        for (auto e : net->ev) (void)hipEventDestroy(e);
        net->ev.clear(); net->ev_kind.clear();
    }
    if (ms_gemm) *ms_gemm = tg / iters;
    if (ms_other) *ms_other = to / iters;
    if (n_gemm) *n_gemm = ng / iters;
    return 0;
}

}
```

### relativepose_amd/model.py

```python
import ctypes as C

import numpy as np
import torch

from . import _lib
from .weights import HEADS, head_channels, parse_output_type, state_dict_spec

PRECISION_CODES = {"f32": 0, "bf16x3": 1, "f16x3": 2, "f16": 3, "bf16x9": 4, "bf16x6": 5}

BUFFER_SHAPES = {"X0": (224, 16), "A1": (224, 192), "A2": (112, 384), "A3": (56, 768), "A4": (28, 256), "A5": (14, 512),
                 "A6": (7, 512), "A7": (3, 512), "A8": (3, 512), "A9": (1, 1024), "D9": (3, 512), "D8": (3, 512),
                 "D7": (7, 512), "D6": (14, 512), "D5": (28, 256), "D4": (56, 128), "D3": (112, 320), "D2": (224, 224)}


_REGISTRY = {}


class SCNet(torch.nn.Module):

    def __init__(self, args):
        super().__init__()
        self.snumclass = int(args.snumclass)
        self.useTanh = int(getattr(args, "useTanh", 1))
        self.batchnorm = int(bool(getattr(args, "batchnorm", 1)))
# ... 107 lines not shown
        self._ws, self._ws_n = ws, n
        return ws

    _tag_counter = 0

    @classmethod
    def new_self_tag(cls):
        cls._tag_counter += 1
        return cls._tag_counter

    FLAG_ZERO_WARP, FLAG_POSE_OUTPUTS = 1, 2

    def forward(self, x, out=None, tail_stream=None, ws_key=None, zero_warp=False, outputs="all", self_tag=0):
        flags = (self.FLAG_ZERO_WARP if zero_warp else 0) | {"all": 0, "pose": self.FLAG_POSE_OUTPUTS}[outputs]
        return self.forward_flags(x, out, flags, self_tag, tail_stream, ws_key)

    def forward_flags(self, x, out=None, flags=0, self_tag=0, tail_stream=None, ws_key=None):
        import torch
        _lib.require_gpu()
        if not self._loaded:
            raise RuntimeError("load_state_dict first")
        assert x.is_cuda and x.dtype == torch.float32 and x.dim() == 4 and x.shape[1] == 16
        x = x.contiguous()
        n, _, H, W = x.shape
        if isinstance(tail_stream, int):
            tail_stream = None if tail_stream == 0 else torch.cuda.ExternalStream(tail_stream)
        ws = self._workspace(n, H, W, x.device, ws_key, tuple(s_ for s_ in (tail_stream,) if s_ is not None))
        if tail_stream is not None:
            x.record_stream(tail_stream)
        user_out = None
        if self.is_variant:
            tail_stream, user_out = None, out
            out = torch.empty(n, self.full_channels, H, W, dtype=torch.float32, device=x.device)
        elif out is None:
            out = torch.empty(n, self.out_channels, H, W, dtype=torch.float32, device=x.device)
            if tail_stream is not None:
                out.record_stream(tail_stream)
        else:
            assert out.is_cuda and out.dtype == torch.float32 and out.is_contiguous() and tuple(out.shape) == (n, self.out_channels, H, W)
        a = _lib.ForwardArgs()
        a.struct_size = C.sizeof(_lib.ForwardArgs)
        a.flags = int(flags) & 3
        a.x, a.out = x.data_ptr(), out.data_ptr()
        a.n_images, a.H, a.W = n, H, W
        a.workspace, a.workspace_bytes = ws.data_ptr(), ws.numel()
        a.stream = torch.cuda.current_stream().cuda_stream
        a.tail_stream = a.stream if tail_stream is None else tail_stream.cuda_stream
        a.self_tag = int(self_tag)
        a.workspace_generation = self._ws_gen
        _lib.check(_lib.lib().relpose_scnet_forward_ex(self._h, C.byref(a)), "relpose_scnet_forward_ex")
        if self.is_variant:
            sel = out if self.out_channels == self.full_channels else out[:, self._sel]
            if user_out is None:
                return sel.contiguous()
            user_out.copy_(sel)
            return user_out
        return out

    def plan_macs(self, n, flags=0, self_cached=False):
        v = C.c_double()
        _lib.check(_lib.lib().relpose_scnet_plan_macs(self._h, int(n), int(flags), 1 if self_cached else 0, C.byref(v)), "relpose_scnet_plan_macs")
        return v.value

    def layer_kernel(self, layer, n):
        r = _lib.lib().relpose_scnet_layer_kernel(self._h, layer.encode(), int(n))
        if r < 0:
            raise KeyError(layer)
        return r

    def zero_tiles(self):
        v = (C.c_int64 * 4)()
        _lib.check(_lib.lib().relpose_scnet_zero_tiles(self._h, _lib.ptr(self._ws), _lib.stream_ptr(), v), "relpose_scnet_zero_tiles")
        return {2: (int(v[0]), int(v[1])), 3: (int(v[2]), int(v[3]))}

    def conv1_zero(self, occupancy=False):
        import numpy as np
        v = (C.c_int64 * 3)()
        occ = np.zeros((self._ws_n, 6, 28), np.uint32) if occupancy else None
        _lib.check(_lib.lib().relpose_scnet_conv1_zero(self._h, _lib.ptr(self._ws), _lib.stream_ptr(), v,
                                                       occ.ctypes.data_as(C.c_void_p) if occupancy else None), "relpose_scnet_conv1_zero")
        counts = (int(v[0]), int(v[1]), int(v[2]))
        return (counts, occ.astype(np.int64)) if occupancy else counts

    def layer_on_strip_kernel(self, layer, n):
        return self.layer_kernel(layer, n) in (1, 2)

    def read_tap(self, name):
        import torch
        L = _lib.lib()
        cnt = L.relpose_scnet_read_tap(self._h, name.encode(), None, None, None)
        if cnt < 0:
            raise KeyError(name)
        H, Cc = BUFFER_SHAPES[name] if name != "OUT" else (224, self.full_channels)
        out = torch.empty(cnt, dtype=torch.float32, device=self._ws.device)
        L.relpose_scnet_read_tap(self._h, name.encode(), _lib.ptr(out), _lib.ptr(self._ws), _lib.stream_ptr())
        return out.view(-1, H, H, Cc)

    def profile(self, x, iters=3):
        import torch
        n, _, H, W = x.shape
        ws = self._workspace(n, H, W, x.device)
        out = torch.empty(n, self.full_channels, H, W, dtype=torch.float32, device=x.device)
        g, o, k = C.c_double(), C.c_double(), C.c_int64()
        rc = _lib.lib().relpose_scnet_profile(self._h, _lib.ptr(x.contiguous()), _lib.ptr(out), n, H, W, _lib.ptr(ws), ws.numel(),
                                              iters, C.byref(g), C.byref(o), C.byref(k), _lib.stream_ptr())
        _lib.check(rc, "relpose_scnet_profile")
        return g.value, o.value, k.value
```

Before: 854.8.

## Compute conv4 split-K slices on a compacted row list, deduplicating empty-neighbourhood rows

Adds a per-pair kernel that marks conv4 output rows whose 3x3 input-block neighbourhood is entirely zero. Each such row is collapsed onto one representative per border class, producing a compacted row list and a remap table. A new ROWS variant of the implicit-GEMM kernel computes only the listed rows for slices where the list is short enough, and the strip kernel then skips those slices. The BN/reduction gathers go through the map. This trades an extra list kernel, an extra launch, and indirection in the reduction for fewer MFMA rows whenever the inputs are sparse.

```diff
diff --git a/include/relpose.h b/include/relpose.h
--- a/include/relpose.h
+++ b/include/relpose.h
@@ -40,7 +40,7 @@
 
 enum { RELPOSE_TUNE_AFFINITY_KERNEL = 0, RELPOSE_TUNE_FIT_MAX_PRODUCTS = 1, RELPOSE_TUNE_FIT_CLUSTER = 2,
        RELPOSE_TUNE_FIT_GLOBAL_VECTORS = 3, RELPOSE_TUNE_FIT_FIXED_CHECKS = 4, RELPOSE_TUNE_HEADS_KERNEL = 5, RELPOSE_TUNE_DECONV_STRIP = 6,
-       RELPOSE_TUNE_ZERO_TILES = 7, RELPOSE_TUNE_CONV1_ZERO = 8, RELPOSE_TUNE_COUNT = 9 };
+       RELPOSE_TUNE_ZERO_TILES = 7, RELPOSE_TUNE_CONV1_ZERO = 8, RELPOSE_TUNE_CONV4_ROWS = 9, RELPOSE_TUNE_COUNT = 10 };
 int relpose_set_tuning(int32_t key, int32_t value);
 const char* relpose_version(void);
 typedef struct RelposeKeypoints {
@@ -595,6 +595,8 @@
 
 int relpose_scnet_conv1_zero(RelposeSCNet* net, void* workspace, void* stream, int64_t* counts_host, uint32_t* occ_host);
 
+int relpose_scnet_conv4_rows(RelposeSCNet* net, void* workspace, void* stream, int64_t* counts_host);
+
 int64_t relpose_scnet_read_tap(RelposeSCNet* net, const char* layer, float* out, void* workspace, void* stream);
 
 int relpose_scnet_profile(RelposeSCNet* net, const float* x, float* out, int32_t n_images, int32_t H, int32_t W,
diff --git a/relativepose_amd/_lib.py b/relativepose_amd/_lib.py
--- a/relativepose_amd/_lib.py
+++ b/relativepose_amd/_lib.py
@@ -266,6 +266,7 @@
     "relpose_scnet_layer_kernel": (c_int, [c_void_p, c_char_p, c_int]),
     "relpose_scnet_zero_tiles": (c_int, [c_void_p, c_void_p, c_void_p, C.POINTER(c_int64)]),
     "relpose_scnet_conv1_zero": (c_int, [c_void_p, c_void_p, c_void_p, C.POINTER(c_int64), c_void_p]),
+    "relpose_scnet_conv4_rows": (c_int, [c_void_p, c_void_p, c_void_p, C.POINTER(c_int64)]),
     "relpose_scnet_read_tap": (c_int64, [c_void_p, c_char_p, c_void_p, c_void_p, c_void_p]),
     "relpose_scnet_profile": (c_int, [c_void_p, c_void_p, c_void_p, c_int, c_int, c_int, c_void_p, c_size_t, c_int,
                                       C.POINTER(c_double), C.POINTER(c_double), C.POINTER(c_int64), c_void_p]),
@@ -309,7 +310,7 @@
 
 
 TUNE_KEYS = {"affinity_kernel": 0, "fit_max_products": 1, "fit_cluster": 2, "fit_global_vectors": 3, "fit_fixed_checks": 4,
-             "heads_kernel": 5, "deconv_strip": 6, "zero_tiles": 7, "conv1_zero": 8}
+             "heads_kernel": 5, "deconv_strip": 6, "zero_tiles": 7, "conv1_zero": 8, "conv4_rows": 9}
 AFFINITY_KERNELS = {"auto": 0, "rows": 1, "tile": 2, "lds": 3, "pool": 4}
 
 
diff --git a/relativepose_amd/csrc/scnet.hip b/relativepose_amd/csrc/scnet.hip
--- a/relativepose_amd/csrc/scnet.hip
+++ b/relativepose_amd/csrc/scnet.hip
@@ -73,6 +73,10 @@
     const int* zt_count;
     const int* zt_list;
     const int2* zt_fill;
+    const int* c4_cnt;
+    const int* c4_list;
+    const int* c4_map;
+    int* c4_hdr;
 };
 
 __device__ __forceinline__ float lrelu(float v, float slope) { return fmaxf(v, slope * v); }
@@ -127,13 +131,19 @@
     }
 }
 
-template <int WM, int WN, int MI, int NI, bool SSLDS, bool UNI = false, int SPLIT = 0>
+__device__ __forceinline__ int rows_tap(int s) {
+    const int p = s >> 3, q = (s >> 2) & 1, ty = (s >> 1) & 1, tx = s & 1;
+    return (p ? 2 * ty : 1 + 2 * ty) * 4 + (q ? 2 * tx : 1 + 2 * tx);
+}
+template <int WM, int WN, int MI, int NI, bool SSLDS, bool UNI = false, int SPLIT = 0, bool ROWS = false>
 __global__ __launch_bounds__(WM * WN * 64, (NI == 4 || SPLIT >= 4) ? 2 : ((WM * WN == 8 || MI == 1) ? 4 : (SSLDS ? 3 : 2))) void conv_igemm_kernel(const ConvDesc* __restrict__ descs, int ninner, int mt_max) {
     constexpr int BM = WM * MI * 32, BN = WN * NI * 32;
+    static_assert(!ROWS || (SSLDS && UNI && SPLIT != 1), "row lists: one BatchNorm group per tile, the strip kernel's operand modes");
     constexpr int LD = RowLd<SPLIT>::v;
     constexpr bool S3 = SPLIT >= 4;
     int zmem, mtile;
-    if (ninner == 1) { zmem = blockIdx.x / mt_max; mtile = blockIdx.x - zmem * mt_max; }
+    if (ROWS) { zmem = 0; mtile = blockIdx.x; }
+    else if (ninner == 1) { zmem = blockIdx.x / mt_max; mtile = blockIdx.x - zmem * mt_max; }
     else {
         const int xcd = blockIdx.x & 7, slot = blockIdx.x >> 3, t8 = (mt_max + 7) >> 3;
         const int inner = slot % ninner, rest = slot / ninner;
@@ -141,6 +151,28 @@
         mtile = (rest % t8) * 8 + xcd;
     }
     const ConvDesc d = descs[zmem];
+    int rows_g = 0, rows_n = 0, rows_t0 = 0;
+    if constexpr (ROWS) {
+        const int G = d.Nimg >> 1, tpg = (2 * d.Hp * d.Wp + BM - 1) / BM;
+        const int ksr = blockIdx.y / d.ntiles_n;
+        int take = 0;
+        for (int q = 0; q < d.ksplit; ++q) {
+            if ((ninner >> q) & 1) continue;
+            const int ng = ((d.shared_slices >> q) & 1) ? 1 : G;
+            int listed = 0, nonfin = 0;
+            for (int g = 0; g < ng; ++g) { const int c = d.c4_cnt[q * G + g]; listed += c & 0x3fffffff; nonfin |= c >> 30; }
+            const bool lp = !nonfin && (long long)listed * 1024 < (long long)mt_max * ng * 2 * d.Hp * d.Wp;
+            take |= lp ? 1 << q : 0;
+            if (blockIdx.x == 0 && blockIdx.y == 0 && threadIdx.x == 0) { d.c4_hdr[2 * q] = listed; d.c4_hdr[2 * q + 1] = lp; }
+        }
+        if (blockIdx.x == 0 && blockIdx.y == 0 && threadIdx.x == 0)
+            *const_cast<int*>(&descs[0].skip_slices) = ninner | take;
+        if (!((take >> ksr) & 1)) return;
+        rows_g = mtile / tpg; rows_t0 = (mtile - rows_g * tpg) * BM;
+        if (((d.shared_slices >> ksr) & 1) && rows_g > 0) return;
+        rows_n = d.c4_cnt[ksr * G + rows_g];
+        if (rows_t0 >= rows_n) return;
+    } else
     if (mtile * BM >= d.M) return;
     constexpr int NT = WM * WN * 64;
     constexpr int RPI = NT / KQ;
@@ -159,12 +191,13 @@
     const int ks = blockIdx.y / d.ntiles_n;
     const int m0 = mtile * BM, n0 = (blockIdx.y - ks * d.ntiles_n) * BN;
     const int hw = d.Hp * d.Wp;
-    const int g0 = (m0 / hw) >> 1;
+    const int g0 = ROWS ? rows_g : (m0 / hw) >> 1;
 
     const int kq = tid % KQ, lrow = tid / KQ;
     int* rtab = reinterpret_cast<int*>(&As[0]);
     for (int row_ = tid; row_ < BM; row_ += NT) {
-        const int m = m0 + row_;
+        int m = m0 + row_;
+        if constexpr (ROWS) m = rows_t0 + row_ < rows_n ? d.c4_list[((size_t)ks * (d.Nimg >> 1) + rows_g) * 2 * hw + rows_t0 + row_] : d.M;
         int pix = -1, base = 0, mg = 0, slot = -1;
         if (m < d.M) {
             const int img = m / hw, rem = m - img * hw;
@@ -175,17 +208,19 @@
             base = (img * d.Hin + y0) * d.Win + x0;
             int msk = 0;
             for (int t = 0; t < d.ntaps; ++t) {
-                const int iy = y0 + descs[zmem].offy[t], ix = x0 + descs[zmem].offx[t];
+                const int to = ROWS ? rows_tap(t) : t;
+                const int iy = y0 + descs[zmem].offy[to], ix = x0 + descs[zmem].offx[to];
                 msk |= ((iy >= 0) & (iy < d.Hin) & (ix >= 0) & (ix < d.Win)) ? (1 << t) : 0;
             }
             mg = msk | ((SSLDS ? ((img >> 1) - g0) * d.Cin : (img >> 1)) << 16);
+            if constexpr (ROWS) pix = m;
         }
         rowpix[row_] = pix; rowslot[row_] = (signed char)slot;
         rtab[2 * row_] = base; rtab[2 * row_ + 1] = mg;
     }
-    if (tid < 16) tapdelta[tid] = (int)descs[zmem].offy[tid] * d.Win + (int)descs[zmem].offx[tid];
+    if (tid < 16) { const int to = ROWS ? rows_tap(tid) : tid; tapdelta[tid] = (int)descs[zmem].offy[to] * d.Win + (int)descs[zmem].offx[to]; }
     if (SSLDS) {
-        const int ng = min(((min(m0 + BM, d.M) - 1) / hw >> 1) - g0 + 1, SS_CAP / d.Cin);
+        const int ng = ROWS ? 1 : min(((min(m0 + BM, d.M) - 1) / hw >> 1) - g0 + 1, SS_CAP / d.Cin);
         for (int idx = tid; idx < ng * d.Cin; idx += NT) {
             const int g = g0 + idx / d.Cin, c = idx % d.Cin;
             const bool s1 = c >= d.src[0].C;
@@ -222,7 +257,8 @@
     const int kt_begin = ks * d.kt_per;
     const int nkt = min(d.K / BK, kt_begin + d.kt_per);
     const int cpt = d.Cin / BK;
-    int tap = d.tap_inner ? kt_begin % d.ntaps : kt_begin / cpt, c0 = (d.tap_inner ? kt_begin / d.ntaps : kt_begin % cpt) * BK;
+    const bool tap_in = ROWS || d.tap_inner;
+    int tap = tap_in ? kt_begin % d.ntaps : kt_begin / cpt, c0 = (tap_in ? kt_begin / d.ntaps : kt_begin % cpt) * BK;
     __syncthreads();
 #pragma unroll
     for (int it = 0; it < A_IT; ++it) {
@@ -259,12 +295,12 @@
             const float* q = reinterpret_cast<const float*>(sss_ + (size_t)g0 * sst_ + cc_);                      \
             qu0 = rp_ldg4(q); qu1 = rp_ldg4(q + 4);                                                               \
         }                                                                                                         \
-        const int kof_ = (tap * d.Cin + c0) * (S3 ? 3 : 2) / 2;                                                   \
+        const int kof_ = ((ROWS ? rows_tap(tap) : tap) * d.Cin + c0) * (S3 ? 3 : 2) / 2;                          \
         _Pragma("unroll") for (int it = 0; it < B_IT; ++it) {                                                     \
             rb[it] = rp_ldg4(b_src[it] + kof_);                                                                   \
             if (S3) { const float2 l_ = rp_ldg2(b_src[it] + kof_ + 32 - kq * 2); rbl[S3 ? it : 0] = l_; }          \
         }                                                                                                         \
-        if (d.tap_inner) { ++tap; if (tap == d.ntaps) { tap = 0; c0 += BK; } }                                    \
+        if (tap_in) { ++tap; if (tap == d.ntaps) { tap = 0; c0 += BK; } }                                         \
         else { c0 += BK; if (c0 == d.Cin) { c0 = 0; ++tap; } }                                                    \
     }
 
@@ -373,7 +409,8 @@
         for (int i = 0; i < MI; ++i)
 #pragma unroll
             for (int r = 0; r < 16; ++r) {
-                const int m = m0 + wm * MI * 32 + i * 32 + (r & 3) + 8 * (r >> 2) + 4 * (lane >> 5);
+                int m = m0 + wm * MI * 32 + i * 32 + (r & 3) + 8 * (r >> 2) + 4 * (lane >> 5);
+                if constexpr (ROWS) { m = rowpix[m - m0]; if (m < 0) continue; }
                 if (m >= d.M) continue;
 #pragma unroll
                 for (int j = 0; j < NI; ++j) rp_stg(po + (size_t)m * d.cout_pad + n0 + wn * NI * 32 + j * 32 + (lane & 31), acc[i][j][r]);
@@ -1450,7 +1487,9 @@
         const int img = m / hw, rem = m - img * hw;
         const int msh = (img & 1) * hw + rem;
         for (int ks = 0; ks < d.ksplit; ++ks) {
-            const float4 v = rp_ldg4(d.partial + ((size_t)ks * d.M + (((d.shared_slices >> ks) & 1) ? msh : m)) * d.cout_pad + c4);
+            int mr = ((d.shared_slices >> ks) & 1) ? msh : m;
+            if (d.c4_map && d.c4_hdr[2 * ks + 1]) mr = d.c4_map[(size_t)ks * d.M + mr];
+            const float4 v = rp_ldg4(d.partial + ((size_t)ks * d.M + mr) * d.cout_pad + c4);
             a.x += v.x; a.y += v.y; a.z += v.z; a.w += v.w;
         }
         const int yp = rem / d.Wp, xp = rem - yp * d.Wp;
@@ -1858,7 +1897,9 @@
             const int img = m / hw, rem = m - img * hw;
             const int msh = (img & 1) * hw + rem;
             for (int ks = 0; ks < d.ksplit; ++ks) {
-                const float4 v = rp_ldg4(d.partial + ((size_t)ks * d.M + (((d.shared_slices >> ks) & 1) ? msh : m)) * d.cout_pad + c4);
+                int mr = ((d.shared_slices >> ks) & 1) ? msh : m;
+                if (d.c4_map && d.c4_hdr[2 * ks + 1]) mr = d.c4_map[(size_t)ks * d.M + mr];
+                const float4 v = rp_ldg4(d.partial + ((size_t)ks * d.M + mr) * d.cout_pad + c4);
                 a.x += v.x; a.y += v.y; a.z += v.z; a.w += v.w;
             }
             const int yp = rem / d.Wp, xp = rem - yp * d.Wp;
@@ -2115,6 +2156,66 @@
     int2* fills = reinterpret_cast<int2*>(zt + ZT_HDR + (size_t)12 * cap) + (size_t)(layer * 6 + q) * cap;
     if (tid < cnt[0] && base[0] + tid < cap) list[base[0] + tid] = comp[tid];
     if (tid < cnt[1] && base[1] + tid < cap) fills[base[1] + tid] = fl[tid];
+}
+
+constexpr int C4R_N = RS / ZT_BLK, C4R_HW = C4R_N * C4R_N;
+static_assert(C4R_N == ZT_NB, "conv4's grid is the occupancy grid");
+constexpr int C4R_THETA_1024 = 717;
+inline size_t c4r_ints(int n) { return 16 + (size_t)6 * (n / 2) + (size_t)12 * n * C4R_HW; }
+__global__ __launch_bounds__(256) void conv4_row_list_kernel(const unsigned* __restrict__ occ, ZtMembers mem, int G, int* __restrict__ cnt,
+                                                             int* __restrict__ list, int* __restrict__ map) {
+    constexpr int R = 2 * C4R_HW, PER = (R + 255) / 256;
+    const int g = blockIdx.x, q = blockIdx.y, tid = threadIdx.x;
+    if (mem.nimg[q] == 0) return;
+    if (2 * g >= mem.nimg[q]) { if (tid == 0) cnt[q * G + g] = 0; return; }
+    __shared__ unsigned ow[2 * ZT_NB];
+    __shared__ int rep[9], nonfin, scan[256];
+    __shared__ unsigned char red[R];
+    if (tid == 0) nonfin = 0;
+    if (tid < 9) rep[tid] = R;
+    __syncthreads();
+    if (tid < 2 * ZT_NB) {
+        const unsigned v = occ[((size_t)(2 * g + tid / ZT_NB) * 6 + q) * ZT_NB + tid % ZT_NB];
+        ow[tid] = v;
+        if (v >> 31) nonfin = 1;
+    }
+    __syncthreads();
+    auto cls_of = [](int r) {
+        const int rem = r % C4R_HW, oy = rem / C4R_N, ox = rem - oy * C4R_N;
+        return 3 * (oy == 0 ? 0 : (oy == C4R_N - 1 ? 2 : 1)) + (ox == 0 ? 0 : (ox == C4R_N - 1 ? 2 : 1));
+    };
+    for (int r = tid; r < R; r += 256) {
+        const int img = r / C4R_HW, rem = r - img * C4R_HW, oy = rem / C4R_N, ox = rem - oy * C4R_N;
+        const int bx0 = max(ox - 1, 0), bx1 = min(ox + 2, C4R_N);
+        const unsigned mask = ((1u << bx1) - 1u) & ~((1u << bx0) - 1u);
+        unsigned any = 0u;
+        for (int by = max(oy - 1, 0); by < min(oy + 2, C4R_N); ++by) any |= ow[img * ZT_NB + by] & mask;
+        const bool rd = any == 0u && !nonfin;
+        red[r] = rd ? 1 : 0;
+        if (rd) atomicMin(&rep[cls_of(r)], r);
+    }
+    __syncthreads();
+    const int r0 = tid * PER, r1 = min(r0 + PER, R);
+    int keep = 0;
+    for (int r = r0; r < r1; ++r) keep += (!red[r] || rep[cls_of(r)] == r) ? 1 : 0;
+    scan[tid] = keep;
+    __syncthreads();
+    for (int off = 1; off < 256; off <<= 1) {
+        const int v = tid >= off ? scan[tid - off] : 0;
+        __syncthreads();
+        scan[tid] += v;
+        __syncthreads();
+    }
+    int pos = scan[tid] - keep;
+    if (tid == 255) cnt[q * G + g] = scan[255] | (nonfin ? 1 << 30 : 0);
+    int* lst = list + ((size_t)q * G + g) * R;
+    int* mp = map + ((size_t)q * G + g) * R;
+    for (int r = r0; r < r1; ++r) {
+        const int rp = rep[cls_of(r)];
+        const bool k = !red[r] || rp == r;
+        if (k) lst[pos++] = g * R + r;
+        mp[r] = g * R + (k ? r : rp);
+    }
 }
 
 template <bool PAIR>
@@ -2333,7 +2434,7 @@
     size_t w1_off = 0;
     size_t wh_off = 0, bh_off = 0;
     std::map<std::pair<void*, int>, void*> plans;
-    struct SelfState { uint64_t tag = 0, gen = 0; int n = 0, H = 0, W = 0; bool pose_only = false; };
+    struct SelfState { uint64_t tag = 0, gen = 0; int n = 0, H = 0, W = 0; bool pose_only = false; bool c4_rows = false; };
     std::map<void*, SelfState> self_state;
     std::map<std::string, Layer> layers;
     std::map<std::string, Buf> bufs;
@@ -2341,6 +2442,8 @@
     size_t gb_floats = 0;
     int last_n = 0;
     const int* last_zt_counts = nullptr;
+    const int* last_c4_hdr = nullptr;
+    int last_c4_nimg[6] = {0, 0, 0, 0, 0, 0};
     int64_t last_zt_units[2] = {0, 0};
     bool w1_finite = false;
     struct A1zState { uint64_t gen = 0; int n = 0, H = 0, W = 0; };
@@ -2603,6 +2706,9 @@
     bool zt = false;
     int zt_nimg[6] = {0, 0, 0, 0, 0, 0};
     int64_t zt_units[2] = {0, 0};
+    bool c4_rows = false;
+    int c4_desc = -1, c4_skip = 0;
+    int c4_nimg[6] = {0, 0, 0, 0, 0, 0};
 };
 
 struct Builder {
@@ -2626,6 +2732,7 @@
     int probe_desc = -1;
     int* zt = nullptr;
     int zt_layer = -1;
+    int* c4r = nullptr;
 
     float* buf(const std::string& b);
     float2* ssb(const std::string& b);
@@ -2878,6 +2985,13 @@
         if (ok) {
             if (shared_slices && (d.Cin / BK) % ksplit == 0) plan->descs[first].shared_slices = shared_slices;
             if (skip_slices && (d.Cin / BK) % ksplit == 0) plan->descs[first].skip_slices = skip_slices;
+            if (c4r && plan->zt && force_ksplit == 6 && ksplit == 6 && d.Cin == 6 * 128 && d.Hp == C4R_N && d.Wp == C4R_N && d.Nimg == n && cp == 256) {
+                ConvDesc& dd = plan->descs[first];
+                const size_t Mr = (size_t)n * C4R_HW;
+                dd.c4_hdr = c4r; dd.c4_cnt = c4r + 16; dd.c4_list = c4r + 16 + 6 * G; dd.c4_map = c4r + 16 + 6 * G + 6 * Mr;
+                plan->c4_rows = true; plan->c4_desc = first; plan->c4_skip = dd.skip_slices;
+                for (int q = 0; q < 6; ++q) plan->c4_nimg[q] = ((dd.skip_slices >> q) & 1) ? 0 : (((dd.shared_slices >> q) & 1) ? 2 : n);
+            }
             Op o; o.type = OP_CONV_STRIP; o.first = first; o.count = 1; o.cfg = 0; o.split = net->prec;
             o.grid = dim3((unsigned)((d.M + 127) / 128), (cp / 128) * ksplit, 1);
             plan->ops.push_back(o);
@@ -3049,7 +3163,7 @@
     net->a1z_state.clear();
 }
 
-struct WsOffsets { size_t act, ss, partial, splitk, statp, persist, snap, zt, total; };
+struct WsOffsets { size_t act, ss, partial, splitk, statp, persist, snap, zt, c4r, total; };
 
 WsOffsets ws_offsets(RelposeSCNet* net, int n) {
     Plan dry;
@@ -3065,6 +3179,7 @@
     o.persist = off; off += rp_align(dry.persist_floats * sizeof(float));
     o.snap = off; off += rp_align(dry.snap_floats * sizeof(float));
     o.zt = off; off += rp_align(zt_ints(n) * sizeof(int));
+    o.c4r = off; off += rp_align(c4r_ints(n) * sizeof(int));
     o.total = off;
     return o;
 }
@@ -3259,15 +3374,17 @@
     const bool pose_only = (flags & RELPOSE_FWD_POSE_OUTPUTS) != 0 && !variant;
     Plan* plan = nullptr;
     RelposeSCNet::SelfState commit;
+    const bool zt_on = g_rp_tune[RELPOSE_TUNE_ZERO_TILES] != 1;
+    const bool c4_on = zt_on && g_rp_tune[RELPOSE_TUNE_CONV4_ROWS] != 1;
+    commit.c4_rows = c4_on;
     commit.tag = self_tag; commit.n = n; commit.H = H; commit.W = W; commit.pose_only = pose_only; commit.gen = ws_gen;
     if (flags & RELPOSE_FWD_NEW_WORKSPACE) net->self_state.erase(workspace);
     RelposeSCNet::SelfState prev = net->self_state[workspace];
     net->self_state[workspace] = RelposeSCNet::SelfState();
     bool self_cached = self_tag != 0 && prev.tag == self_tag && prev.n == n && prev.H == H && prev.W == W && prev.pose_only == pose_only && !zero_warp &&
-                       prev.gen == ws_gen;
+                       prev.gen == ws_gen && prev.c4_rows == c4_on;
     int snap_mode = 0;
-    const bool zt_on = g_rp_tune[RELPOSE_TUNE_ZERO_TILES] != 1;
-    const int ds_key = ((g_rp_tune[RELPOSE_TUNE_DECONV_STRIP] == 1 ? 1 : 0) << 28) | ((zt_on ? 0 : 1) << 29);
+    const int ds_key = ((g_rp_tune[RELPOSE_TUNE_DECONV_STRIP] == 1 ? 1 : 0) << 28) | ((zt_on ? 0 : 1) << 29) | ((c4_on ? 0 : 1) << 30);
     for (int attempt = 0; attempt < 2 && !plan; ++attempt) {
         snap_mode = self_cached ? 2 : (self_tag != 0 ? 1 : 0);
         const int plan_key = (int)n | (zero_warp ? 1 << 24 : 0) | (pose_only ? 1 << 25 : 0) | (self_cached ? 1 << 26 : 0) | (snap_mode == 1 ? 1 << 27 : 0) | ds_key;
@@ -3288,6 +3405,7 @@
         B.persist = (float*)(ws + o.persist);
         B.snapbuf = (float*)(ws + o.snap); B.snap_mode = snap_mode; p->snap_mode = snap_mode;
         B.zt = zt_on ? (int*)(ws + o.zt) + zt_occ_ints(n) : nullptr;
+        B.c4r = c4_on ? (int*)(ws + o.c4r) : nullptr;
         build_plan(net, n, B);
         if (B.rc) {
             delete p;
@@ -3339,7 +3457,7 @@
     else
         hipLaunchKernelGGL(resize_in_kernel, dim3(2048), dim3(256), 0, s, x, act + net->bufs["X0"].off * n, n, H, W, plan->self_cached ? 8 : 0);
     mark(-3);
-    net->last_zt_counts = nullptr;
+    net->last_zt_counts = nullptr; net->last_c4_hdr = nullptr;
     net->last_zt_units[0] = plan->zt_units[0]; net->last_zt_units[1] = plan->zt_units[1];
     net->last_c1_units = 0; net->last_c1_codes = false; net->last_occ = plan->zt;
     if (plan->zt) {
@@ -3349,6 +3467,15 @@
         if (!occ_fused)
             hipLaunchKernelGGL(x0_occupancy_kernel, dim3(n * ZT_NB), dim3(256), 0, s, act + net->bufs["X0"].off * n, occ, ztp, plan->self_cached ? 8 : 0);
         hipLaunchKernelGGL(zero_tile_list_kernel, dim3(G, 6, 2), dim3(128), 0, s, occ, ztp, zm, n * ZT_PPI);
+        if (plan->c4_rows) {
+            const ConvDesc& d4 = plan->descs[plan->c4_desc];
+            ZtMembers cm;
+            for (int q = 0; q < 6; ++q) cm.nimg[q] = plan->c4_nimg[q];
+            hipLaunchKernelGGL(conv4_row_list_kernel, dim3(G, 6), dim3(256), 0, s, occ, cm, G, const_cast<int*>(d4.c4_cnt), const_cast<int*>(d4.c4_list),
+                               const_cast<int*>(d4.c4_map));
+            net->last_c4_hdr = d4.c4_hdr;
+            for (int q = 0; q < 6; ++q) net->last_c4_nimg[q] = plan->c4_nimg[q];
+        }
         mark(-2);
         net->last_zt_counts = ztp;
     }
@@ -3423,7 +3550,16 @@
 #define RP_L_STRIP(SP_) hipLaunchKernelGGL((conv_s2_strip_kernel<4, SP_>), op.grid, dim3(256), 0, s, plan->d_descs + op.first)
 #define RP_L_DSTRIP(SP_) hipLaunchKernelGGL((deconv_strip_kernel<4, SP_>), op.grid, dim3(256), 0, s, plan->d_descs + op.first, op.mt_max)
             if (op.cfg == 1) RP_TILE_SPLIT(RP_L_DSTRIP);
-            else RP_TILE_SPLIT(RP_L_STRIP);
+            else {
+                if (plan->c4_rows && op.first == plan->c4_desc) {
+                    const dim3 rg((unsigned)(G * ((2 * C4R_HW + 127) / 128)), op.grid.y, 1);
+                    const int theta = g_rp_tune[RELPOSE_TUNE_CONV4_ROWS] == 2 ? (1 << 20) : C4R_THETA_1024;
+#define RP_L_ROWS(SP_) hipLaunchKernelGGL((conv_igemm_kernel<2, 2, 2, 2, true, true, SP_, true>), rg, dim3(256), 0, s, plan->d_descs + op.first, plan->c4_skip, theta)
+                    RP_TILE_SPLIT(RP_L_ROWS);
+#undef RP_L_ROWS
+                }
+                RP_TILE_SPLIT(RP_L_STRIP);
+            }
 #undef RP_L_STRIP
 #undef RP_L_DSTRIP
             mark(-1);
@@ -3638,6 +3774,27 @@
     return 0;
 }
 
+int relpose_scnet_conv4_rows(RelposeSCNet* net, void* workspace, void* stream, int64_t* counts_host) {
+    if (!net || !net->finalized || !workspace || !counts_host || net->last_n <= 0) return RELPOSE_EINVAL;
+    for (int i = 0; i < 18; ++i) counts_host[i] = 0;
+    if (!net->last_c4_hdr) {
+        counts_host[0] = -1;
+        return 0;
+    }
+    const char* lo = (const char*)workspace + ws_offsets(net, net->last_n).c4r;
+    if ((const char*)net->last_c4_hdr != lo) return RELPOSE_EINVAL;
+    int h[12];
+    RP_HIP(hipMemcpyAsync(h, net->last_c4_hdr, sizeof(h), hipMemcpyDeviceToHost, (hipStream_t)stream));
+    RP_HIP(hipStreamSynchronize((hipStream_t)stream));
+    for (int q = 0; q < 6; ++q) {
+        const int64_t rows = (int64_t)net->last_c4_nimg[q] * C4R_HW;
+        if (rows == 0) continue;
+        const bool lp = h[2 * q + 1] != 0;
+        counts_host[3 * q] = lp ? h[2 * q] : rows; counts_host[3 * q + 1] = lp ? rows - h[2 * q] : 0; counts_host[3 * q + 2] = lp ? 1 : 0;
+    }
+    return 0;
+}
+
 int relpose_scnet_conv1_zero(RelposeSCNet* net, void* workspace, void* stream, int64_t* counts_host, uint32_t* occ_host) {
     if (!net || !net->finalized || !workspace || !counts_host || net->last_n <= 0) return RELPOSE_EINVAL;
     const int n = net->last_n;
diff --git a/relativepose_amd/model.py b/relativepose_amd/model.py
--- a/relativepose_amd/model.py
+++ b/relativepose_amd/model.py
@@ -213,6 +213,13 @@
         counts = (int(v[0]), int(v[1]), int(v[2]))
         return (counts, occ.astype(np.int64)) if occupancy else counts
 
+    def conv4_rows(self):
+        v = (C.c_int64 * 18)()
+        _lib.check(_lib.lib().relpose_scnet_conv4_rows(self._h, _lib.ptr(self._ws), _lib.stream_ptr(), v), "relpose_scnet_conv4_rows")
+        if v[0] < 0:
+            return None
+        return [(int(v[3 * q]), int(v[3 * q + 1]), bool(v[3 * q + 2])) for q in range(6)]
+
     def layer_on_strip_kernel(self, layer, n):
         return self.layer_kernel(layer, n) in (1, 2)
 
```

After: 879.4, median of 6. +2.9%, better.
